# szy4017/DeepSense6G_TII

Hardware: NVIDIA B200
Metric: train samples/sec (fwd+bwd) (higher is better)
Workload: dtype bf16

## Files before the change

### deepsense6g_tii_b200/csrc/attn_api.cu

```cuda
#include <algorithm>
#include <atomic>

#include "tc_common.cuh"

namespace dsf {


__global__ void __launch_bounds__(256)
attn_delta_kernel(const __nv_bfloat16* __restrict__ y, const __nv_bfloat16* __restrict__ dy, float* __restrict__ delta, int B, int T,
                  int C, int nh) {
  pdl_trigger();
  pdl_wait();
  const int lane = threadIdx.x & 31;
  const int hs = C / nh, gl = hs / 8;
  const int nchunk = C / 8;
  for (int64_t row = (int64_t)blockIdx.x * 8 + (threadIdx.x >> 5); row < (int64_t)B * T; row += (int64_t)gridDim.x * 8) {
    const int b = (int)(row / T), t = (int)(row % T);
    for (int c0 = 0; c0 < nchunk; c0 += 32) {
      const int ch = c0 + lane;
      float acc = 0.f;
      if (ch < nchunk) {
        const uint4 a = __ldg(reinterpret_cast<const uint4*>(y + row * C + ch * 8));
        const uint4 d = __ldg(reinterpret_cast<const uint4*>(dy + row * C + ch * 8));
        const __nv_bfloat162* ap = reinterpret_cast<const __nv_bfloat162*>(&a);
        const __nv_bfloat162* dp = reinterpret_cast<const __nv_bfloat162*>(&d);
#pragma unroll
        for (int k = 0; k < 4; ++k) {
          const float2 af = __bfloat1622float2(ap[k]), df = __bfloat1622float2(dp[k]);
          acc += af.x * df.x + af.y * df.y;
        }
      }
      for (int o = gl >> 1; o > 0; o >>= 1) acc += __shfl_xor_sync(0xffffffffu, acc, o);
      if (ch < nchunk && (lane % gl) == 0) delta[((size_t)b * nh + (ch * 8) / hs) * T + t] = acc;
    }
  }
}

int attn_fwd_run(const void* qkv, void* y, float* lse, int B, int T, int C, int nh, const dsf_dropout* drop, uint32_t* bits, int force_nwg,
                 cudaStream_t st);
int attn_bwd_run(const void* qkv, const void* y, const void* dy, const float* lse, float* delta, void* dqkv, int B, int T, int C, int nh,
                 const dsf_dropout* drop, uint32_t* bits, int parts, cudaStream_t st);

int run_attn_delta(const void* y, const void* dy, float* delta, int B, int T, int C, int nh, cudaStream_t st) {
  launch_pdl(attn_delta_kernel, dim3(std::min(cdiv(B * T, 8), num_sms() * 8)), dim3(256), 0, st, (const __nv_bfloat16*)y, (const __nv_bfloat16*)dy,
             delta, B, T, C, nh);
  return check_launch("attn_bwd/delta");
}

static std::atomic<int> g_attn_impl{0};

}

using namespace dsf;

extern "C" int dsf_attn_set_impl(int32_t impl) {
  DSF_REQUIRE(impl >= 0 && impl <= 2, "attn_set_impl: impl must be 0 (default), 1 (128-row forward CTAs) or 2 (256-row forward CTAs)");
  g_attn_impl.store(impl, std::memory_order_relaxed);
  return DSF_OK;
}

static int check_attn_drop(const char* who, const dsf_dropout* drop, const uint32_t* bits, bool& on) {
  on = drop && drop->p > 0.f;
  if (!on) return DSF_OK;
  if (!(drop->p < 1.f)) { set_error("%s: dropout p must be in [0, 1)", who); return DSF_EINVAL; }
  if (!bits) { set_error("%s: attention dropout needs the drop_bits buffer", who); return DSF_EINVAL; }
  return DSF_OK;
}

static int check_head_size(const char* who, int hs) {
  if (hs == 16 || hs == 32 || hs == 64 || hs == 128) return DSF_OK;
  set_error("%s: head size %d not supported (16, 32, 64, 128)", who, hs);
  return DSF_EUNSUPPORTED;
}

extern "C" int64_t dsf_attn_drop_words(int32_t B, int32_t T, int32_t nh) {
  if (B <= 0 || T <= 0 || nh <= 0) return 0;
  return (int64_t)B * nh * T * (2 * cdiv(T, 64));
}

extern "C" int dsf_attn_fwd(const void* qkv, void* y, float* lse, int32_t B, int32_t T, int32_t C, int32_t nh, const dsf_dropout* drop,
                            uint32_t* drop_bits, void* stream) {
  DSF_REQUIRE(qkv && y && lse, "attn_fwd: NULL pointer");
  bool drop_on;
  if (int e = check_attn_drop("attn_fwd", drop, drop_bits, drop_on)) return e;
  DSF_REQUIRE(B > 0 && T > 0 && C > 0 && nh > 0 && C % nh == 0, "attn_fwd: bad shape B=%d T=%d C=%d nh=%d", B, T, C, nh);
  DSF_REQUIRE(aligned16(qkv) && aligned16(y), "attn_fwd: 16-byte alignment required");
  DSF_REQUIRE(B <= 65535 && nh <= 65535, "attn_fwd: grid too large");
  if (int e = check_head_size("attn_fwd", C / nh)) return e;
  return attn_fwd_run(qkv, y, lse, B, T, C, nh, drop_on ? drop : nullptr, drop_bits, g_attn_impl.load(std::memory_order_relaxed), (cudaStream_t)stream);
}

static int attn_bwd_impl(const void* qkv, const void* y, const void* dy, const float* lse, float* delta, void* dqkv, int32_t B, int32_t T,
                         int32_t C, int32_t nh, const dsf_dropout* drop, const uint32_t* drop_bits, int parts, void* stream) {
  DSF_REQUIRE(qkv && y && dy && lse && delta && dqkv, "attn_bwd: NULL pointer");
  bool drop_on;
  if (int e = check_attn_drop("attn_bwd", drop, drop_bits, drop_on)) return e;
  DSF_REQUIRE(B > 0 && T > 0 && C > 0 && nh > 0 && C % nh == 0, "attn_bwd: bad shape B=%d T=%d C=%d nh=%d", B, T, C, nh);
  DSF_REQUIRE(aligned16(qkv) && aligned16(y) && aligned16(dy) && aligned16(dqkv), "attn_bwd: 16-byte alignment required");
  DSF_REQUIRE(B <= 65535 && nh <= 65535, "attn_bwd: grid too large");
  if (int e = check_head_size("attn_bwd", C / nh)) return e;
  return attn_bwd_run(qkv, y, dy, lse, delta, dqkv, B, T, C, nh, drop_on ? drop : nullptr, const_cast<uint32_t*>(drop_bits), parts, (cudaStream_t)stream);
}

extern "C" int dsf_attn_bwd(const void* qkv, const void* y, const void* dy, const float* lse, float* delta, void* dqkv, int32_t B,
                            int32_t T, int32_t C, int32_t nh, const dsf_dropout* drop, const uint32_t* drop_bits, void* stream) {
  return attn_bwd_impl(qkv, y, dy, lse, delta, dqkv, B, T, C, nh, drop, drop_bits, 7, stream);
}

extern "C" int dsf_attn_bwd_parts(const void* qkv, const void* y, const void* dy, const float* lse, float* delta, void* dqkv, int32_t B,
                                  int32_t T, int32_t C, int32_t nh, const dsf_dropout* drop, const uint32_t* drop_bits, int32_t parts,
                                  void* stream) {
  DSF_REQUIRE(parts > 0 && parts <= 7, "attn_bwd_parts: parts must be a non-empty subset of {1 = delta, 2 = dK/dV, 4 = dQ}");
  return attn_bwd_impl(qkv, y, dy, lse, delta, dqkv, B, T, C, nh, drop, drop_bits, parts, stream);
}
```

### deepsense6g_tii_b200/csrc/attn_tc2.cu

```cuda
#include <algorithm>
#include <cstdlib>

#include "tc_common.cuh"

namespace dsf {

using namespace tc;

__device__ __forceinline__ void tma_load_3d(uint32_t dst, const CUtensorMap* m, uint32_t bar, int c0, int c1, int c2) {
  asm volatile(
      "cp.async.bulk.tensor.3d.shared::cluster.global.mbarrier::complete_tx::bytes [%0], [%1, {%3, %4, %5}], [%2];" ::"r"(dst),
      "l"(reinterpret_cast<uint64_t>(m)), "r"(bar), "r"(c0), "r"(c1), "r"(c2)
      : "memory");
}
#ifdef DSF_ATTN_TRACE
__device__ long long g_attn_trace[3][64][6];
#define TRACE(who, it, slot)                                                                               \
  do {                                                                                                     \
    if (blockIdx.x == 0 && blockIdx.y == 0 && blockIdx.z == 0 && (threadIdx.x & 31) == 0 && (it) < 64)     \
      g_attn_trace[who][it][slot] = clock64();                                                             \
  } while (0)
#else
#define TRACE(who, it, slot) do {} while (0)
#endif

__device__ __forceinline__ float ex2_approx(float x) {
  float y;
  asm("ex2.approx.ftz.f32 %0, %1;" : "=f"(y) : "f"(x));
  return y;
}
__device__ __forceinline__ uint64_t pack2(float lo, float hi) { uint64_t r; asm("mov.b64 %0, {%1, %2};" : "=l"(r) : "f"(lo), "f"(hi)); return r; }
__device__ __forceinline__ void unpack2(uint64_t v, float& lo, float& hi) { asm("mov.b64 {%0, %1}, %2;" : "=f"(lo), "=f"(hi) : "l"(v)); }
__device__ __forceinline__ uint64_t fma2(uint64_t a, uint64_t b, uint64_t c) { uint64_t d; asm("fma.rn.f32x2 %0, %1, %2, %3;" : "=l"(d) : "l"(a), "l"(b), "l"(c)); return d; }
__device__ __forceinline__ uint64_t add2(uint64_t a, uint64_t b) { uint64_t d; asm("add.rn.f32x2 %0, %1, %2;" : "=l"(d) : "l"(a), "l"(b)); return d; }
__device__ __forceinline__ uint64_t mul2(uint64_t a, uint64_t b) { uint64_t d; asm("mul.rn.f32x2 %0, %1, %2;" : "=l"(d) : "l"(a), "l"(b)); return d; }
__device__ __forceinline__ void ex2_poly2(uint64_t x, float& p0, float& p1) {
  float x0, x1;
  unpack2(x, x0, x1);
  const uint64_t xc = pack2(fmaxf(x0, -126.f), fmaxf(x1, -126.f));
  const uint64_t t = add2(xc, pack2(12582912.f, 12582912.f));
  const uint64_t r = add2(t, pack2(-12582912.f, -12582912.f));
  const uint64_t f = fma2(r, pack2(-1.f, -1.f), xc);
  uint64_t q = fma2(f, pack2(0.05517164617776871f, 0.05517164617776871f), pack2(0.2426111251115799f, 0.2426111251115799f));
  q = fma2(q, f, pack2(0.6932609677314758f, 0.6932609677314758f));
  q = fma2(q, f, pack2(0.9999280571937561f, 0.9999280571937561f));
  float q0, q1, t0, t1;
  unpack2(q, q0, q1);
  unpack2(t, t0, t1);
  p0 = __int_as_float(__float_as_int(q0) + (__float_as_int(t0) << 23));
  p1 = __int_as_float(__float_as_int(q1) + (__float_as_int(t1) << 23));
}

template <int POLY>
__device__ __forceinline__ uint64_t ex2_pair(uint64_t x, int j) {
  float p0, p1;
  if (POLY > 0 && (j % (POLY > 0 ? POLY : 1)) == POLY - 1) {
    ex2_poly2(x, p0, p1);
  } else {
    float x0, x1;
    unpack2(x, x0, x1);
    p0 = ex2_approx(x0);
    p1 = ex2_approx(x1);
  }
  return pack2(p0, p1);
}
__device__ __forceinline__ uint32_t pack_bf16x2_pair(uint64_t v) {
  float lo, hi;
  unpack2(v, lo, hi);
  return pack_bf16x2(lo, hi);
}

struct AttnDrop {
  uint32_t thresh8;
  float scale;
  uint32_t k0, k1, site;
  uint32_t* bits;
  int Tw;
  const unsigned long long* seed_dev;
};
__device__ __forceinline__ uint32_t attn_keep_word(const AttnDrop& a, uint64_t rowid, uint32_t word) {
  uint32_t out = 0;
  const uint32_t t4 = a.thresh8 * 0x01010101u;
#pragma unroll
  for (int c = 0; c < 2; ++c) {
    const uint4 r = philox4x32(a.k0, a.k1, (uint32_t)rowid, (uint32_t)(rowid >> 32), word * 2 + c, a.site);
    const uint32_t w[4] = {r.x, r.y, r.z, r.w};
#pragma unroll
    for (int k = 0; k < 4; ++k) {
      const uint32_t ge = __vcmpgeu4(w[k], t4) & 0x01010101u;
      out |= (((ge * 0x01020408u) >> 24) & 0xFu) << (c * 16 + k * 4);
    }
  }
  return out;
}
__device__ __forceinline__ void named_bar_sync(int id, int nthreads) {
  asm volatile("bar.sync %0, %1;" ::"r"(id), "r"(nthreads) : "memory");
}
__device__ __forceinline__ void named_bar_arrive(int id, int nthreads) {
  asm volatile("bar.arrive %0, %1;" ::"r"(id), "r"(nthreads) : "memory");
}

template <int HS>
struct HeadCfg {
  static constexpr int BOXC = HS < 64 ? HS : 64;
  static constexpr int ROWB = BOXC * 2;
  static constexpr int NHALF = HS / BOXC;
  static constexpr uint32_t SWZ = ROWB == 128 ? SWZ_128B : (ROWB == 64 ? SWZ_64B : SWZ_32B);
  static constexpr int KPH = ROWB / 32;
};

template <int HS>
__device__ __forceinline__ uint64_t kmaj_desc(uint32_t tile, int R, int kk) {
  using H = HeadCfg<HS>;
  const uint32_t off = (uint32_t)(kk / H::KPH) * R * H::ROWB + (uint32_t)(kk % H::KPH) * 32;
  return make_smem_desc(tile + off, 16, 8 * H::ROWB, H::SWZ);
}
template <int HS>
__device__ __forceinline__ uint64_t mnmaj_desc(uint32_t tile, int R, int kk) {
  using H = HeadCfg<HS>;
  return make_smem_desc(tile + (uint32_t)kk * 16 * H::ROWB, (uint32_t)R * H::ROWB, 8 * H::ROWB, H::SWZ);
}
template <int KC>
__device__ __forceinline__ uint64_t pdesc(uint32_t tile, int kk) {
  return make_smem_desc(tile + (uint32_t)kk * 256, 128, KC * 16, SWZ_NONE);
}

__device__ __forceinline__ void tc_commit_elect(uint32_t bar) {
  if (elect_one()) tc::tc_commit(bar);
  __syncwarp();
}
template <int HS>
__device__ __forceinline__ void mma_over_head(uint32_t tmem_d, uint32_t a_tile, int RA, uint32_t b_tile, int RB, uint32_t idesc) {
  using H = HeadCfg<HS>;
  const uint64_t da = make_smem_desc(a_tile, 16, 8 * H::ROWB, H::SWZ), db = make_smem_desc(b_tile, 16, 8 * H::ROWB, H::SWZ);
  if (elect_one()) {
#pragma unroll
    for (int kk = 0; kk < HS / 16; ++kk) {
      const uint32_t oa = (uint32_t)(kk / H::KPH) * RA * H::ROWB + (uint32_t)(kk % H::KPH) * 32;
      const uint32_t ob = (uint32_t)(kk / H::KPH) * RB * H::ROWB + (uint32_t)(kk % H::KPH) * 32;
      tc_mma_bf16(tmem_d, da + (oa >> 4), db + (ob >> 4), idesc, kk != 0);
    }
  }
  __syncwarp();
}
template <int HS, int KC>
__device__ __forceinline__ void mma_over_rows(uint32_t tmem_d, uint32_t p_tile, uint32_t b_tile, uint32_t idesc, bool accumulate) {
  using H = HeadCfg<HS>;
  const uint64_t dp = make_smem_desc(p_tile, 128, KC * 16, SWZ_NONE);
  const uint64_t db = make_smem_desc(b_tile, (uint32_t)KC * H::ROWB, 8 * H::ROWB, H::SWZ);
  const uint32_t acc = accumulate ? 1u : 0u;
  if (elect_one()) {
#pragma unroll
    for (int kk = 0; kk < KC / 16; ++kk)
      tc_mma_bf16(tmem_d, dp + (uint32_t)((kk * 256) >> 4), db + (uint32_t)((kk * 16 * H::ROWB) >> 4), idesc, kk == 0 ? acc : 1u);
  }
  __syncwarp();
}

template <int HS, int KC, int CW = 0>
__device__ __forceinline__ void mma_over_rows_ts(uint32_t tmem_d, uint32_t p_tmem, uint32_t b_tile, uint32_t idesc, bool accumulate) {
  using H = HeadCfg<HS>;
  const uint64_t db = make_smem_desc(b_tile, (uint32_t)KC * H::ROWB, 8 * H::ROWB, H::SWZ);
  const uint32_t acc = accumulate ? 1u : 0u;
  if (elect_one()) {
#pragma unroll
    for (int kk = 0; kk < KC / 16; ++kk) {
      const uint32_t col = CW > 0 ? (uint32_t)((kk * 16 / (CW > 0 ? CW : 1)) * CW + (kk * 16 % (CW > 0 ? CW : 1)) / 2) : (uint32_t)(kk * 8);
      tc_mma_bf16_ts(tmem_d, p_tmem + col, db + (uint32_t)((kk * 16 * H::ROWB) >> 4), idesc, kk == 0 ? acc : 1u);
    }
  }
  __syncwarp();
}

template <int HS>
__device__ __forceinline__ void mma_over_head_ts(uint32_t tmem_d, uint32_t a_tmem, uint32_t b_tile, int RB, uint32_t idesc) {
  using H = HeadCfg<HS>;
  const uint64_t db = make_smem_desc(b_tile, 16, 8 * H::ROWB, H::SWZ);
  if (elect_one()) {
#pragma unroll
    for (int kk = 0; kk < HS / 16; ++kk) {
      const uint32_t ob = (uint32_t)(kk / H::KPH) * RB * H::ROWB + (uint32_t)(kk % H::KPH) * 32;
      tc_mma_bf16_ts(tmem_d, a_tmem + (uint32_t)(kk * 8), db + (ob >> 4), idesc, kk != 0);
    }
  }
  __syncwarp();
}

template <int HS>
__device__ __forceinline__ void tma_tile(uint32_t dst, const CUtensorMap* m, uint32_t bar, int col0, int row0, int b, int R) {
  using H = HeadCfg<HS>;
#pragma unroll
  for (int hf = 0; hf < H::NHALF; ++hf) tma_load_3d(dst + hf * R * H::ROWB, m, bar, col0 + hf * H::BOXC, row0, b);
}

template <int KC>
__device__ __forceinline__ void store_p32(uint8_t* tile, int row, int c, const uint32_t (&pk)[16]) {
#pragma unroll
  for (int cc = 0; cc < 4; ++cc) {
    uint8_t* dst = tile + ((size_t)(row >> 3) * (KC / 8) + (c >> 3) + cc) * 128 + (row & 7) * 16;
    *reinterpret_cast<uint4*>(dst) = make_uint4(pk[4 * cc], pk[4 * cc + 1], pk[4 * cc + 2], pk[4 * cc + 3]);
  }
}

__device__ __forceinline__ void store_row16_bf16(__nv_bfloat16* dst, const uint32_t (&a)[16], float scale) {
#pragma unroll
  for (int e = 0; e < 16; e += 8)
    *reinterpret_cast<uint4*>(dst + e) =
        make_uint4(pack_bf16x2(__uint_as_float(a[e]) * scale, __uint_as_float(a[e + 1]) * scale),
                   pack_bf16x2(__uint_as_float(a[e + 2]) * scale, __uint_as_float(a[e + 3]) * scale),
                   pack_bf16x2(__uint_as_float(a[e + 4]) * scale, __uint_as_float(a[e + 5]) * scale),
                   pack_bf16x2(__uint_as_float(a[e + 6]) * scale, __uint_as_float(a[e + 7]) * scale));
}

template <int HS, int BQ, int ST, int NP>
struct BwdKV2 {
  static constexpr int KV_BYTES = 128 * HS * 2, Q_BYTES = BQ * HS * 2;
  static constexpr int K_OFF = 0, V_OFF = KV_BYTES, Q_OFF = 2 * KV_BYTES, DO_OFF = Q_OFF + ST * Q_BYTES;
  static constexpr int BAR_OFF = DO_OFF + ST * Q_BYTES;
  static constexpr int NBAR = 2 + 2 * ST + 4;
  static constexpr int STAT_OFF = BAR_OFF + NBAR * 8 + 16;
  static constexpr int THREADS = 256 * NP + 64;
  static_assert(4 * BQ + 2 * HS <= 512, "TMEM budget");
  static_assert(STAT_OFF % 16 == 0, "float4 reads of the statistics");
  static int dyn_bytes(int T) { return STAT_OFF + 2 * cdiv(T, BQ) * BQ * 4 + 1024; }
};

template <int HS, int BQ, int ST, int NP, bool DROP, int POLY>
__global__ void __launch_bounds__(256 * NP + 64, 1)
attn_bwd_kv2_kernel(const __grid_constant__ CUtensorMap tmKV, const __grid_constant__ CUtensorMap tmQ, const __grid_constant__ CUtensorMap tmDO,
                    const float* __restrict__ lse, const float* __restrict__ delta, __nv_bfloat16* __restrict__ dqkv, int T, int C, int nh,
                    float scale, AttnDrop ad) {
  using L = BwdKV2<HS, BQ, ST, NP>;
  constexpr int MMAW = 8 * NP, TMAW = 8 * NP + 1;
  extern __shared__ uint8_t smem_raw[];
  const uint32_t sbase = (smem_u32(smem_raw) + 1023u) & ~1023u;
  uint8_t* smem = smem_raw + (sbase - smem_u32(smem_raw));
  const uint32_t bar0 = sbase + L::BAR_OFF;
  const uint32_t kv_full = bar0, acc_done = bar0 + 8, q_full = bar0 + 16, q_empty = q_full + 8 * ST, s_full = q_empty + 8 * ST,
                 ds_full = s_full + 16, tmem_slot = ds_full + 16;
  const int warp = __shfl_sync(0xffffffffu, (int)(threadIdx.x >> 5), 0), lane = threadIdx.x & 31;
  const int kv0 = blockIdx.x * 128, h = blockIdx.y, b = blockIdx.z;
  const int n_q = (T + BQ - 1) / BQ;

  pdl_trigger();
  if (threadIdx.x == 0) {
    mbar_init(kv_full, 1);
    mbar_init(acc_done, 1);
    for (int s = 0; s < ST; ++s) { mbar_init(q_full + 8 * s, 1); mbar_init(q_empty + 8 * s, 1); }
    for (int w = 0; w < 2; ++w) { mbar_init(s_full + 8 * w, 1); mbar_init(ds_full + 8 * w, 256 * NP); }
    fence_barrier_init();
  }
  if (warp == MMAW) { tmem_alloc(tmem_slot, 512); tmem_relinquish(); }
  if (warp == TMAW && lane == 0) { tma_prefetch_desc(&tmKV); tma_prefetch_desc(&tmQ); tma_prefetch_desc(&tmDO); }
  tc_fence_before();
  __syncthreads();
  tc_fence_after();
  uint32_t tmem_base;
  asm volatile("ld.shared.b32 %0, [%1];" : "=r"(tmem_base) : "r"(tmem_slot));
  pdl_wait();
  const uint32_t tm_dv = tmem_base + 4 * BQ, tm_dk = tm_dv + HS;

  if (warp == TMAW) {
    if (lane == 0) {
      mbar_expect_tx(kv_full, 2 * L::KV_BYTES);
      tma_tile<HS>(sbase + L::K_OFF, &tmKV, kv_full, C + h * HS, kv0, b, 128);
      tma_tile<HS>(sbase + L::V_OFF, &tmKV, kv_full, 2 * C + h * HS, kv0, b, 128);
      for (int i = 0; i < n_q; ++i) {
        const int st = i % ST;
        if (i >= ST) mbar_wait(q_empty + 8 * st, ((i / ST) - 1) & 1);
        mbar_expect_tx(q_full + 8 * st, 2 * L::Q_BYTES);
        tma_tile<HS>(sbase + L::Q_OFF + st * L::Q_BYTES, &tmQ, q_full + 8 * st, h * HS, i * BQ, b, BQ);
        tma_tile<HS>(sbase + L::DO_OFF + st * L::Q_BYTES, &tmDO, q_full + 8 * st, h * HS, i * BQ, b, BQ);
      }
    }
  } else if (warp == MMAW) {
    {
      constexpr uint32_t idesc_s = make_idesc_bf16(128, BQ, 0, 0);
      constexpr uint32_t idesc_g = make_idesc_bf16(128, HS, 0, 1);
      mbar_wait(kv_full, 0);
      mbar_wait(q_full, 0);
      tc_fence_after();
      mma_over_head<HS>(tmem_base, sbase + L::K_OFF, 128, sbase + L::Q_OFF, BQ, idesc_s);
      mma_over_head<HS>(tmem_base + BQ, sbase + L::V_OFF, 128, sbase + L::DO_OFF, BQ, idesc_s);
      tc_commit_elect(s_full);
      for (int i = 0; i < n_q; ++i) {
        const int bf = i & 1, st = i % ST;
        TRACE(2, i, 0);
        if (i + 1 < n_q) {
          const int sn = (i + 1) % ST, bn = (i + 1) & 1;
          mbar_wait(q_full + 8 * sn, ((i + 1) / ST) & 1);
          TRACE(2, i, 1);
          tc_fence_after();
          mma_over_head<HS>(tmem_base + bn * 2 * BQ, sbase + L::K_OFF, 128, sbase + L::Q_OFF + sn * L::Q_BYTES, BQ, idesc_s);
          mma_over_head<HS>(tmem_base + bn * 2 * BQ + BQ, sbase + L::V_OFF, 128, sbase + L::DO_OFF + sn * L::Q_BYTES, BQ, idesc_s);
          tc_commit_elect(s_full + 8 * bn);
        }
        TRACE(2, i, 2);
        mbar_wait(ds_full + 8 * bf, (i >> 1) & 1);
        TRACE(2, i, 3);
        tc_fence_after();
        mma_over_rows_ts<HS, BQ, 32 / NP>(tm_dv, tmem_base + bf * 2 * BQ, sbase + L::DO_OFF + st * L::Q_BYTES, idesc_g, i > 0);
        mma_over_rows_ts<HS, BQ, 32 / NP>(tm_dk, tmem_base + bf * 2 * BQ + BQ, sbase + L::Q_OFF + st * L::Q_BYTES, idesc_g, i > 0);
        tc_commit_elect(q_empty + 8 * st);
        TRACE(2, i, 4);
      }
      tc_commit_elect(acc_done);
    }
  } else {
    constexpr int CW = BQ / (2 * NP);
    const int wgi = warp >> 2;
    const int row = (warp & 3) * 32 + lane;
    const uint32_t lane_off = (uint32_t)((warp & 3) * 32) << 16;
    const bool key_ok = (kv0 + row) < T;
    const float scale_log2 = scale * 1.4426950408889634f;
    const float* lse_g = lse + ((size_t)b * nh + h) * T;
    const float* delta_g = delta + ((size_t)b * nh + h) * T;
    static_assert(BQ == 64 && (CW == 32 || CW == 16), "a 64-query tile in 32- or 16-column shares");
    const size_t bh = (size_t)b * nh + h;
    const int kw = kv0 / 32 + (warp & 3);
    float* s_lse = reinterpret_cast<float*>(smem + L::STAT_OFF);
    float* s_delta = s_lse + n_q * BQ;
    for (int idx = threadIdx.x; idx < n_q * BQ; idx += 256 * NP) {
      s_lse[idx] = idx < T ? __ldg(lse_g + idx) * -1.4426950408889634f : -INFINITY;
      s_delta[idx] = idx < T ? -__ldg(delta_g + idx) : 0.f;
    }
    uint32_t wv = 0xFFFFFFFFu;
    auto fetch_w = [&](int it) {
      const int qq = it * BQ + wgi * CW + (lane % CW);
      wv = qq < T ? ad.bits[(bh * T + qq) * ad.Tw + kw] : 0u;
    };
    if (DROP) fetch_w(0);
    named_bar_sync(1, 256 * NP);
    for (int i = 0; i < n_q; ++i) {
      const int bf = i & 1;
      const float* wst = s_lse + i * BQ + wgi * CW;
      const float* wsd = s_delta + i * BQ + wgi * CW;
      const uint32_t myw = wv;
      if ((warp & 3) == 0 && wgi < 2) TRACE(wgi, i, 0);
      if (DROP && i + 1 < n_q) fetch_w(i + 1);
      if ((warp & 3) == 0 && wgi < 2) TRACE(wgi, i, 1);
      mbar_wait(s_full + 8 * bf, (i >> 1) & 1);
      if ((warp & 3) == 0 && wgi < 2) TRACE(wgi, i, 2);
      tc_fence_after();
      const uint32_t tm_s = tmem_base + bf * 2 * BQ + lane_off + wgi * CW, tm_dp = tm_s + BQ;
      uint32_t rs[CW], rp[CW];
      if constexpr (CW == 32) { tmem_ld32(tm_s, rs); tmem_ld32(tm_dp, rp); }
      else { tmem_ld16(tm_s, rs); tmem_ld16(tm_dp, rp); }
      tmem_wait_ld();
      if ((warp & 3) == 0 && wgi < 2) TRACE(wgi, i, 3);
      const uint64_t sc2 = pack2(scale_log2, scale_log2);
#pragma unroll
      for (int c = 0; c < CW; c += 16) {
        uint32_t pk[8], dk[8];
#pragma unroll
        for (int e = 0; e < 16; e += 4) {
          if (!DROP) {
            const ulonglong2 nl = *reinterpret_cast<const ulonglong2*>(wst + c + e);
            const ulonglong2 nd = *reinterpret_cast<const ulonglong2*>(wsd + c + e);
#pragma unroll
            for (int u = 0; u < 4; u += 2) {
              const uint64_t x = fma2(pack2(__uint_as_float(rs[c + e + u]), __uint_as_float(rs[c + e + u + 1])), sc2, u ? nl.y : nl.x);
              const uint64_t p2 = ex2_pair<POLY>(x, (c + e + u) / 2);
              const uint64_t t2 = add2(pack2(__uint_as_float(rp[c + e + u]), __uint_as_float(rp[c + e + u + 1])), u ? nd.y : nd.x);
              pk[(e + u) / 2] = pack_bf16x2_pair(p2);
              dk[(e + u) / 2] = pack_bf16x2_pair(mul2(p2, t2));
            }
            continue;
          }
          const float4 l4 = *reinterpret_cast<const float4*>(wst + c + e);
          const float4 d4 = *reinterpret_cast<const float4*>(wsd + c + e);
          const float ls[4] = {l4.x, l4.y, l4.z, l4.w}, dl[4] = {d4.x, d4.y, d4.z, d4.w};
          float p[4], d[4];
#pragma unroll
          for (int u = 0; u < 4; ++u) {
            p[u] = ex2_approx(fmaf(__uint_as_float(rs[c + e + u]), scale_log2, ls[u]));
            float dp = __uint_as_float(rp[c + e + u]);
            const float m = (__shfl_sync(0xffffffffu, myw, c + e + u) >> lane) & 1u ? ad.scale : 0.f;
            dp *= m;
            d[u] = p[u] * (dp + dl[u]);
            p[u] *= m;
          }
          pk[e / 2] = pack_bf16x2(p[0], p[1]);
          pk[e / 2 + 1] = pack_bf16x2(p[2], p[3]);
          dk[e / 2] = pack_bf16x2(d[0], d[1]);
          dk[e / 2 + 1] = pack_bf16x2(d[2], d[3]);
        }
        tmem_st8(tm_s + c / 2, pk);
        tmem_st8(tm_dp + c / 2, dk);
      }
      if ((warp & 3) == 0 && wgi < 2) TRACE(wgi, i, 4);
      tmem_wait_st();
      tc_fence_before();
      mbar_arrive(ds_full + 8 * bf);
      if ((warp & 3) == 0 && wgi < 2) TRACE(wgi, i, 5);
    }
    mbar_wait(acc_done, 0);
    tc_fence_after();
    const int ld = 3 * C;
    __nv_bfloat16* dk_row = dqkv + ((size_t)b * T + kv0 + row) * ld + C + h * HS;
    __nv_bfloat16* dv_row = dk_row + C;
    constexpr int NSPLIT = (NP == 2 && HS >= 32) ? 2 : 1;
    constexpr int CH = HS / NSPLIT;
    const int which = wgi & 1, part = wgi >> 1;
    if (part < NSPLIT) {
#pragma unroll 1
      for (int c = part * CH; c < (part + 1) * CH; c += 16) {
        uint32_t a[16];
        tmem_ld16((which == 0 ? tm_dk : tm_dv) + lane_off + c, a);
        tmem_wait_ld();
        if (key_ok) store_row16_bf16((which == 0 ? dk_row : dv_row) + c, a, which == 0 ? scale : 1.0f);
      }
    }
  }
  tc_fence_before();
  __syncthreads();
  if (warp == MMAW) tmem_dealloc(tmem_base, 512);
}

template <int HS, int ST>
struct BwdQ2 {
  static constexpr int BKV = 64;
  static constexpr int Q_BYTES = 128 * HS * 2, KV_BYTES = BKV * HS * 2;
  static constexpr int Q_OFF = 0, DO_OFF = Q_BYTES, K_OFF = 2 * Q_BYTES, V_OFF = K_OFF + ST * KV_BYTES;
  static constexpr int BAR_OFF = V_OFF + ST * KV_BYTES;
  static constexpr int NBAR = 2 + 2 * ST + 4;
  static constexpr int DYN = BAR_OFF + NBAR * 8 + 16 + 1024;
  static_assert(4 * BKV + HS <= 512, "TMEM budget");
};

template <int HS, int ST, bool AT, int NP, bool DROP, int POLY>
__global__ void __launch_bounds__(256 * NP + 64, 1)
attn_bwd_q2_kernel(const __grid_constant__ CUtensorMap tmQ, const __grid_constant__ CUtensorMap tmDO, const __grid_constant__ CUtensorMap tmKV,
                   const float* __restrict__ lse, const float* __restrict__ delta, __nv_bfloat16* __restrict__ dqkv, int T, int C, int nh,
                   float scale, AttnDrop ad, const __nv_bfloat16* __restrict__ qkv, const __nv_bfloat16* __restrict__ dy) {
  using L = BwdQ2<HS, ST>;
  constexpr int BKV = L::BKV;
  constexpr int MMAW = 8 * NP, TMAW = 8 * NP + 1;
  extern __shared__ uint8_t smem_raw[];
  const uint32_t sbase = (smem_u32(smem_raw) + 1023u) & ~1023u;
  const uint32_t bar0 = sbase + L::BAR_OFF;
  const uint32_t q_full = bar0, acc_done = bar0 + 8, kv_full = bar0 + 16, kv_empty = kv_full + 8 * ST, s_full = kv_empty + 8 * ST,
                 ds_full = s_full + 16, tmem_slot = ds_full + 16;
  const int warp = __shfl_sync(0xffffffffu, (int)(threadIdx.x >> 5), 0), lane = threadIdx.x & 31;
  const int q0 = blockIdx.x * 128, h = blockIdx.y, b = blockIdx.z;
  const int n_kv = (T + BKV - 1) / BKV;
  constexpr uint32_t TMEM_COLS = (4 * BKV + HS + (AT ? (HS >= 32 ? HS : 32) : 0)) <= 256 ? 256 : 512;
  static_assert(4 * BKV + 2 * HS <= 512, "TMEM budget (S/dP double-buffered, dQ, Q and dO rows)");

  pdl_trigger();
  if (threadIdx.x == 0) {
    mbar_init(q_full, AT ? 256 : 1);
    mbar_init(acc_done, 1);
    for (int s = 0; s < ST; ++s) { mbar_init(kv_full + 8 * s, 1); mbar_init(kv_empty + 8 * s, 1); }
    for (int w = 0; w < 2; ++w) { mbar_init(s_full + 8 * w, 1); mbar_init(ds_full + 8 * w, 256 * NP); }
    fence_barrier_init();
  }
  if (warp == MMAW) { tmem_alloc(tmem_slot, TMEM_COLS); tmem_relinquish(); }
  if (warp == TMAW && lane == 0) { tma_prefetch_desc(&tmKV); tma_prefetch_desc(&tmQ); tma_prefetch_desc(&tmDO); }
  tc_fence_before();
  __syncthreads();
  tc_fence_after();
  uint32_t tmem_base;
  asm volatile("ld.shared.b32 %0, [%1];" : "=r"(tmem_base) : "r"(tmem_slot));
  pdl_wait();
  const uint32_t tm_dq = tmem_base + 4 * BKV;
  const uint32_t tm_q = tm_dq + HS, tm_do = tm_q + (HS >= 32 ? HS / 2 : 16);

  if (warp == TMAW) {
    if (lane == 0) {
      if (!AT) {
        mbar_expect_tx(q_full, 2 * L::Q_BYTES);
        tma_tile<HS>(sbase + L::Q_OFF, &tmQ, q_full, h * HS, q0, b, 128);
        tma_tile<HS>(sbase + L::DO_OFF, &tmDO, q_full, h * HS, q0, b, 128);
      }
      for (int j = 0; j < n_kv; ++j) {
        const int st = j % ST;
        if (j >= ST) mbar_wait(kv_empty + 8 * st, ((j / ST) - 1) & 1);
        mbar_expect_tx(kv_full + 8 * st, 2 * L::KV_BYTES);
        tma_tile<HS>(sbase + L::K_OFF + st * L::KV_BYTES, &tmKV, kv_full + 8 * st, C + h * HS, j * BKV, b, BKV);
        tma_tile<HS>(sbase + L::V_OFF + st * L::KV_BYTES, &tmKV, kv_full + 8 * st, 2 * C + h * HS, j * BKV, b, BKV);
      }
    }
  } else if (warp == MMAW) {
    {
      constexpr uint32_t idesc_s = make_idesc_bf16(128, BKV, 0, 0);
      constexpr uint32_t idesc_q = make_idesc_bf16(128, HS, 0, 1);
      mbar_wait(q_full, 0);
      mbar_wait(kv_full, 0);
      tc_fence_after();
      if (AT) {
        mma_over_head_ts<HS>(tmem_base, tm_q, sbase + L::K_OFF, BKV, idesc_s);
        mma_over_head_ts<HS>(tmem_base + BKV, tm_do, sbase + L::V_OFF, BKV, idesc_s);
      } else {
        mma_over_head<HS>(tmem_base, sbase + L::Q_OFF, 128, sbase + L::K_OFF, BKV, idesc_s);
        mma_over_head<HS>(tmem_base + BKV, sbase + L::DO_OFF, 128, sbase + L::V_OFF, BKV, idesc_s);
      }
      tc_commit_elect(s_full);
      for (int j = 0; j < n_kv; ++j) {
        const int bf = j & 1, st = j % ST;
        if (j + 1 < n_kv) {
          const int sn = (j + 1) % ST, bn = (j + 1) & 1;
          mbar_wait(kv_full + 8 * sn, ((j + 1) / ST) & 1);
          tc_fence_after();
          if (AT) {
            mma_over_head_ts<HS>(tmem_base + bn * 2 * BKV, tm_q, sbase + L::K_OFF + sn * L::KV_BYTES, BKV, idesc_s);
            mma_over_head_ts<HS>(tmem_base + bn * 2 * BKV + BKV, tm_do, sbase + L::V_OFF + sn * L::KV_BYTES, BKV, idesc_s);
          } else {
            mma_over_head<HS>(tmem_base + bn * 2 * BKV, sbase + L::Q_OFF, 128, sbase + L::K_OFF + sn * L::KV_BYTES, BKV, idesc_s);
            mma_over_head<HS>(tmem_base + bn * 2 * BKV + BKV, sbase + L::DO_OFF, 128, sbase + L::V_OFF + sn * L::KV_BYTES, BKV, idesc_s);
          }
          tc_commit_elect(s_full + 8 * bn);
        }
        mbar_wait(ds_full + 8 * bf, (j >> 1) & 1);
        tc_fence_after();
        mma_over_rows_ts<HS, BKV, 32 / NP>(tm_dq, tmem_base + bf * 2 * BKV + BKV, sbase + L::K_OFF + st * L::KV_BYTES, idesc_q, j > 0);
        tc_commit_elect(kv_empty + 8 * st);
      }
      tc_commit_elect(acc_done);
    }
  } else {
    constexpr int CW = BKV / (2 * NP);
    static_assert(BKV == 64 && (CW == 32 || CW == 16), "a 64-key tile in 32- or 16-column shares");
    const int wgi = warp >> 2;
    const int row = (warp & 3) * 32 + lane;
    const uint32_t lane_off = (uint32_t)((warp & 3) * 32) << 16;
    const int q = q0 + row;
    const bool q_ok = q < T;
    const float scale_log2 = scale * 1.4426950408889634f;
    const float my_lse = q_ok ? lse[((size_t)b * nh + h) * T + q] * 1.4426950408889634f : INFINITY;
    const float my_delta = q_ok ? delta[((size_t)b * nh + h) * T + q] : 0.f;
    if (AT && wgi < 2) {
      const __nv_bfloat16* src = wgi == 0 ? qkv + ((size_t)b * T + q) * (3 * C) + h * HS : dy + ((size_t)b * T + q) * C + h * HS;
      const uint32_t dst = (wgi == 0 ? tm_q : tm_do) + lane_off;
#pragma unroll 1
      for (int c = 0; c < HS; c += 32) {
        uint32_t wds[16];
#pragma unroll
        for (int k = 0; k < 4; ++k) {
          const bool real = q_ok && (HS >= 32 || k < 2);
          const uint4 v = real ? __ldg(reinterpret_cast<const uint4*>(src + c) + k) : make_uint4(0u, 0u, 0u, 0u);
          wds[4 * k] = v.x; wds[4 * k + 1] = v.y; wds[4 * k + 2] = v.z; wds[4 * k + 3] = v.w;
        }
        tmem_st16(dst + c / 2, wds);
      }
      tmem_wait_st();
      tc_fence_before();
      mbar_arrive(q_full);
    }
    const uint32_t* my_bits = (DROP && q_ok) ? ad.bits + (((size_t)b * nh + h) * T + q) * ad.Tw + (wgi * CW) / 32 : nullptr;
    uint32_t wnext = my_bits ? my_bits[0] : 0xFFFFFFFFu;
    for (int j = 0; j < n_kv; ++j) {
      const int bf = j & 1, kv0 = j * BKV;
      const uint32_t keepw = wnext >> ((wgi * CW) % 32);
      if (my_bits && j + 1 < n_kv) wnext = my_bits[2 * (j + 1)];
      mbar_wait(s_full + 8 * bf, (j >> 1) & 1);
      tc_fence_after();
      const uint32_t tm_s = tmem_base + bf * 2 * BKV + lane_off + wgi * CW, tm_dp = tm_s + BKV;
      const bool full = kv0 + BKV <= T;
      uint32_t rs[CW], rp[CW];
      if constexpr (CW == 32) { tmem_ld32(tm_s, rs); tmem_ld32(tm_dp, rp); }
      else { tmem_ld16(tm_s, rs); tmem_ld16(tm_dp, rp); }
      tmem_wait_ld();
#pragma unroll
      for (int c = 0; c < CW; c += 16) {
        uint32_t dk[8];
        if (full && !DROP) {
          const uint64_t sc2 = pack2(scale_log2, scale_log2), nl2 = pack2(-my_lse, -my_lse), nd2 = pack2(-my_delta, -my_delta);
#pragma unroll
          for (int e = 0; e < 16; e += 2) {
            const uint64_t x = fma2(pack2(__uint_as_float(rs[c + e]), __uint_as_float(rs[c + e + 1])), sc2, nl2);
            const uint64_t p2 = ex2_pair<POLY>(x, (c + e) / 2);
            const uint64_t t2 = add2(pack2(__uint_as_float(rp[c + e]), __uint_as_float(rp[c + e + 1])), nd2);
            dk[e / 2] = pack_bf16x2_pair(mul2(p2, t2));
          }
        } else {
          const int k0 = kv0 + wgi * CW + c;
#pragma unroll
          for (int e = 0; e < 16; e += 2) {
            float p0 = (k0 + e < T) ? ex2_approx(fmaf(__uint_as_float(rs[c + e]), scale_log2, -my_lse)) : 0.f;
            float p1 = (k0 + e + 1 < T) ? ex2_approx(fmaf(__uint_as_float(rs[c + e + 1]), scale_log2, -my_lse)) : 0.f;
            float dp0 = __uint_as_float(rp[c + e]), dp1 = __uint_as_float(rp[c + e + 1]);
            if (DROP) {
              dp0 *= (keepw >> (c + e)) & 1u ? ad.scale : 0.f;
              dp1 *= (keepw >> (c + e + 1)) & 1u ? ad.scale : 0.f;
            }
            dk[e / 2] = pack_bf16x2(p0 * (dp0 - my_delta), p1 * (dp1 - my_delta));
          }
        }
        tmem_st8(tm_dp + c / 2, dk);
      }
      tmem_wait_st();
      tc_fence_before();
      mbar_arrive(ds_full + 8 * bf);
    }
    mbar_wait(acc_done, 0);
    tc_fence_after();
    __nv_bfloat16* dq_row = dqkv + ((size_t)b * T + q) * (3 * C) + h * HS;
    constexpr int NG = (HS / 16) < 2 * NP ? (HS / 16) : 2 * NP;
    constexpr int CH = HS / NG;
    const int g = wgi;
    if (g < NG) {
#pragma unroll 1
      for (int c = g * CH; c < (g + 1) * CH; c += 16) {
        uint32_t a[16];
        tmem_ld16(tm_dq + lane_off + c, a);
        tmem_wait_ld();
        if (q_ok) store_row16_bf16(dq_row + c, a, scale);
      }
    }
  }
  tc_fence_before();
  __syncthreads();
  if (warp == MMAW) tmem_dealloc(tmem_base, TMEM_COLS);
}

template <int HS, int KST, int VST, int NWG = 2, bool PT = false>
struct Fwd3 {
  static constexpr int BKV = 64;
  static constexpr int Q_BYTES = 128 * HS * 2, KV_BYTES = BKV * HS * 2, P_BYTES = 128 * BKV * 2;
  static constexpr int Q_OFF = 0, K_OFF = NWG * Q_BYTES, V_OFF = K_OFF + KST * KV_BYTES, P_OFF = V_OFF + VST * KV_BYTES;
  static constexpr int BAR_OFF = P_OFF + (PT ? 0 : 2 * NWG * P_BYTES);
  static constexpr int NBAR = 1 + 2 * KST + 2 * VST + 12;
  static constexpr int DYN = BAR_OFF + NBAR * 8 + 16 + 1024;
  static constexpr int THREADS = 128 * NWG + 64;
  static constexpr int MIN_CTAS = NWG == 1 ? 2 : 1;
  static constexpr uint32_t TMEM_COLS = NWG == 1 ? 256 : 512;
  static_assert(2 * NWG * BKV + NWG * HS <= (int)TMEM_COLS, "TMEM budget");
  static_assert(DYN <= 232448 / MIN_CTAS - 1024 * (MIN_CTAS - 1), "shared memory budget");
};

template <int HS, int KST, int VST, bool PT, bool PP, int NWG = 2, int POLY = 0>
__global__ void __launch_bounds__(128 * NWG + 64, NWG == 1 ? 2 : 1)
attn_fwd3_kernel(const __grid_constant__ CUtensorMap tmQ, const __grid_constant__ CUtensorMap tmKV, __nv_bfloat16* __restrict__ y,
                 float* __restrict__ lse, int T, int C, int nh, float scale_log2, AttnDrop ad) {
  using L = Fwd3<HS, KST, VST, NWG, PT>;
  constexpr int BKV = L::BKV;
  constexpr int MMAW = 4 * NWG, TMAW = 4 * NWG + 1;
  static_assert(!PP || NWG == 2, "ping-pong needs two warpgroups");
  extern __shared__ uint8_t smem_raw[];
  const uint32_t sbase = (smem_u32(smem_raw) + 1023u) & ~1023u;
  uint8_t* smem = smem_raw + (sbase - smem_u32(smem_raw));
  const uint32_t bar0 = sbase + L::BAR_OFF;
  const uint32_t q_full = bar0, k_full = bar0 + 8, k_empty = k_full + 8 * KST, v_full = k_empty + 8 * KST, v_empty = v_full + 8 * VST,
                 s_full = v_empty + 8 * VST, p_full = s_full + 32, p_empty = p_full + 32, tmem_slot = p_empty + 32;
  const int warp = __shfl_sync(0xffffffffu, (int)(threadIdx.x >> 5), 0), lane = threadIdx.x & 31;
  const int q0 = blockIdx.x * (128 * NWG), h = blockIdx.y, b = blockIdx.z;
  const int n_kv = (T + BKV - 1) / BKV;

  pdl_trigger();
  if (threadIdx.x == 0) {
    mbar_init(q_full, 1);
    for (int s = 0; s < KST; ++s) { mbar_init(k_full + 8 * s, 1); mbar_init(k_empty + 8 * s, 1); }
    for (int s = 0; s < VST; ++s) { mbar_init(v_full + 8 * s, 1); mbar_init(v_empty + 8 * s, 1); }
    for (int i = 0; i < 2 * NWG; ++i) { mbar_init(s_full + 8 * i, 1); mbar_init(p_full + 8 * i, 128); mbar_init(p_empty + 8 * i, 1); }
    fence_barrier_init();
  }
  if (warp == MMAW) { tmem_alloc(tmem_slot, L::TMEM_COLS); tmem_relinquish(); }
  if (warp == TMAW && lane == 0) { tma_prefetch_desc(&tmQ); tma_prefetch_desc(&tmKV); }
  tc_fence_before();
  __syncthreads();
  tc_fence_after();
  uint32_t tmem_base;
  asm volatile("ld.shared.b32 %0, [%1];" : "=r"(tmem_base) : "r"(tmem_slot));
  pdl_wait();
  if (ad.thresh8 && ad.seed_dev != nullptr) {
    const unsigned long long sd = __ldg(ad.seed_dev);
    ad.k0 ^= (uint32_t)(sd & 0xFFFFFFFFull);
    ad.k1 ^= (uint32_t)(sd >> 32);
  }

  if (warp == TMAW) {
    if (lane == 0) {
      mbar_expect_tx(q_full, NWG * L::Q_BYTES);
      for (int w = 0; w < NWG; ++w) tma_tile<HS>(sbase + L::Q_OFF + w * L::Q_BYTES, &tmQ, q_full, h * HS, q0 + 128 * w, b, 128);
      for (int j = 0; j < n_kv; ++j) {
        const int ks = j % KST, vs = j % VST;
        if (j >= KST) mbar_wait(k_empty + 8 * ks, ((j / KST) - 1) & 1);
        mbar_expect_tx(k_full + 8 * ks, L::KV_BYTES);
        tma_tile<HS>(sbase + L::K_OFF + ks * L::KV_BYTES, &tmKV, k_full + 8 * ks, C + h * HS, j * BKV, b, BKV);
        if (j >= VST) mbar_wait(v_empty + 8 * vs, ((j / VST) - 1) & 1);
        mbar_expect_tx(v_full + 8 * vs, L::KV_BYTES);
        tma_tile<HS>(sbase + L::V_OFF + vs * L::KV_BYTES, &tmKV, v_full + 8 * vs, 2 * C + h * HS, j * BKV, b, BKV);
      }
    }
  } else if (warp == MMAW) {
    {
      constexpr uint32_t idesc_s = make_idesc_bf16(128, BKV, 0, 0);
      constexpr uint32_t idesc_o = make_idesc_bf16(128, HS, 0, 1);
      mbar_wait(q_full, 0);
      for (int jj = 0; jj < 2 && jj < n_kv; ++jj) {
        mbar_wait(k_full + 8 * (jj % KST), (jj / KST) & 1);
        tc_fence_after();
        for (int w = 0; w < NWG; ++w) {
          mma_over_head<HS>(tmem_base + (w * 2 + jj) * BKV, sbase + L::Q_OFF + w * L::Q_BYTES, 128, sbase + L::K_OFF + (jj % KST) * L::KV_BYTES,
                            BKV, idesc_s);
          tc_commit_elect(s_full + 8 * (w * 2 + jj));
        }
        tc_commit_elect(k_empty + 8 * (jj % KST));
      }
      for (int j = 0; j < n_kv; ++j) {
        const int buf = j & 1, vs = j % VST;
        TRACE(2, j, 0);
        mbar_wait(v_full + 8 * vs, (j / VST) & 1);
        for (int w = 0; w < NWG; ++w) {
          const int sb = w * 2 + buf;
          TRACE(2, j, 1 + 2 * w);
          mbar_wait(p_full + 8 * sb, (j >> 1) & 1);
          TRACE(2, j, 2 + 2 * w);
          tc_fence_after();
          if (PT)
            mma_over_rows_ts<HS, BKV>(tmem_base + 2 * NWG * BKV + w * HS, tmem_base + sb * BKV, sbase + L::V_OFF + vs * L::KV_BYTES, idesc_o, j > 0);
          else
            mma_over_rows<HS, BKV>(tmem_base + 2 * NWG * BKV + w * HS, sbase + L::P_OFF + sb * L::P_BYTES, sbase + L::V_OFF + vs * L::KV_BYTES, idesc_o,
                                   j > 0);
          tc_commit_elect(p_empty + 8 * sb);
          if (w == NWG - 1) tc_commit_elect(v_empty + 8 * vs);
          if (j + 2 < n_kv) {
            const int ks = (j + 2) % KST;
            if (w == 0) { mbar_wait(k_full + 8 * ks, ((j + 2) / KST) & 1); tc_fence_after(); }
            mma_over_head<HS>(tmem_base + sb * BKV, sbase + L::Q_OFF + w * L::Q_BYTES, 128, sbase + L::K_OFF + ks * L::KV_BYTES, BKV, idesc_s);
            tc_commit_elect(s_full + 8 * sb);
            if (w == NWG - 1) tc_commit_elect(k_empty + 8 * ks);
          }
        }
      }
    }
  } else {
    const int w = warp >> 2;
    const int row = (warp & 3) * 32 + lane;
    const uint32_t lane_off = (uint32_t)((warp & 3) * 32) << 16;
    const uint32_t tm_o = tmem_base + 2 * NWG * BKV + w * HS + lane_off;
    float m_run = -INFINITY, l_run = 0.f;
    if (PP && w == 1) named_bar_arrive(3, 256);
    for (int j = 0; j < n_kv; ++j) {
      const int kv0 = j * BKV, buf = j & 1, sb = w * 2 + buf;
      const uint32_t tm_s = tmem_base + sb * BKV + lane_off;
      uint8_t* p_tile = smem + L::P_OFF + sb * L::P_BYTES;
      if ((warp & 3) == 0) TRACE(w, j, 0);
      mbar_wait(s_full + 8 * sb, (j >> 1) & 1);
      if ((warp & 3) == 0) TRACE(w, j, 1);
      tc_fence_after();
      uint32_t r0[32], r1[32];
      tmem_ld32(tm_s, r0);
      tmem_ld32(tm_s + 32, r1);
      tmem_wait_ld();
      if ((warp & 3) == 0) TRACE(w, j, 2);
      float p_max = -INFINITY;
      if (kv0 + BKV <= T) {
        float m4[4] = {-INFINITY, -INFINITY, -INFINITY, -INFINITY};
#pragma unroll
        for (int i = 0; i < 32; ++i) m4[i & 3] = fmaxf(m4[i & 3], fmaxf(__uint_as_float(r0[i]), __uint_as_float(r1[i])));
        p_max = fmaxf(fmaxf(m4[0], m4[1]), fmaxf(m4[2], m4[3]));
      } else {
#pragma unroll
        for (int i = 0; i < 32; ++i) {
          if (kv0 + i < T) p_max = fmaxf(p_max, __uint_as_float(r0[i]));
          if (kv0 + 32 + i < T) p_max = fmaxf(p_max, __uint_as_float(r1[i]));
        }
      }
      p_max *= scale_log2;
      const bool need = p_max > m_run + 8.f;
      if (__any_sync(0xffffffffu, need)) {
        const float m_new = need ? p_max : m_run;
        const float alpha = ex2_approx(m_run - m_new);
        if (j > 0) {
          mbar_wait(p_empty + 8 * (w * 2 + ((j - 1) & 1)), ((j - 1) >> 1) & 1);
          tc_fence_after();
#pragma unroll 1
          for (int c = 0; c < HS; c += 16) {
            uint32_t o[16];
            tmem_ld16(tm_o + c, o);
            tmem_wait_ld();
#pragma unroll
            for (int i = 0; i < 16; ++i) o[i] = __float_as_uint(__uint_as_float(o[i]) * alpha);
            tmem_st16(tm_o + c, o);
          }
          tmem_wait_st();
        }
        l_run *= alpha;
        m_run = m_new;
      }
      if ((warp & 3) == 0) TRACE(w, j, 3);
      if (!PT && j >= 2) mbar_wait(p_empty + 8 * sb, ((j >> 1) - 1) & 1);
      if (PP) named_bar_sync(3 + w, 256);
      if ((warp & 3) == 0) TRACE(w, j, 4);
      float l_add = 0.f;
      const bool full = kv0 + BKV <= T;
      const int qrow = q0 + 128 * w + row;
      const uint64_t rowid = ((uint64_t)b * nh + h) * T + qrow;
      if (POLY > 0 && PT && full && !ad.thresh8) {
        const uint64_t sc2 = pack2(scale_log2, scale_log2), nm2 = pack2(-m_run, -m_run);
        uint64_t lsum = pack2(0.f, 0.f);
#pragma unroll
        for (int half = 0; half < 2; ++half) {
          uint32_t pk[16];
#pragma unroll
          for (int i = 0; i < 32; i += 2) {
            const uint32_t a0 = half ? r1[i] : r0[i], a1 = half ? r1[i + 1] : r0[i + 1];
            const uint64_t x = fma2(pack2(__uint_as_float(a0), __uint_as_float(a1)), sc2, nm2);
            float p0, p1;
            if (((i / 2) % (POLY > 0 ? POLY : 1)) == POLY - 1) {
              ex2_poly2(x, p0, p1);
            } else {
              float x0, x1;
              unpack2(x, x0, x1);
              p0 = ex2_approx(x0);
              p1 = ex2_approx(x1);
            }
            lsum = add2(lsum, pack2(p0, p1));
            pk[i / 2] = pack_bf16x2(p0, p1);
          }
          tmem_st16(tm_s + half * 16, pk);
        }
        float l0, l1;
        unpack2(lsum, l0, l1);
        l_add = l0 + l1;
      } else
#pragma unroll
      for (int half = 0; half < 2; ++half) {
        uint32_t keepw = 0xFFFFFFFFu;
        if (ad.thresh8) {
          keepw = attn_keep_word(ad, rowid, (uint32_t)(kv0 / 32 + half));
          if (qrow < T) ad.bits[rowid * ad.Tw + kv0 / 32 + half] = keepw;
        }
        uint32_t pk[16];
#pragma unroll
        for (int i = 0; i < 32; i += 2) {
          const uint32_t a0 = half ? r1[i] : r0[i], a1 = half ? r1[i + 1] : r0[i + 1];
          float p0 = ex2_approx(fmaf(__uint_as_float(a0), scale_log2, -m_run));
          float p1 = ex2_approx(fmaf(__uint_as_float(a1), scale_log2, -m_run));
          if (!full) {
            if (kv0 + half * 32 + i >= T) p0 = 0.f;
            if (kv0 + half * 32 + i + 1 >= T) p1 = 0.f;
          }
          l_add += p0 + p1;
          if (ad.thresh8) {
            p0 *= (keepw >> i) & 1u ? ad.scale : 0.f;
            p1 *= (keepw >> (i + 1)) & 1u ? ad.scale : 0.f;
          }
          pk[i / 2] = pack_bf16x2(p0, p1);
        }
        if (PT) tmem_st16(tm_s + half * 16, pk);
        else store_p32<BKV>(p_tile, row, half * 32, pk);
      }
      if (PP) named_bar_arrive(4 - w, 256);
      l_run += l_add;
      if (PT) tmem_wait_st();
      else fence_proxy_async();
      tc_fence_before();
      mbar_arrive(p_full + 8 * sb);
      if ((warp & 3) == 0) TRACE(w, j, 5);
    }
    mbar_wait(p_empty + 8 * (w * 2 + ((n_kv - 1) & 1)), ((n_kv - 1) >> 1) & 1);
    tc_fence_after();
    const int q = q0 + 128 * w + row;
    const float inv_l = 1.0f / l_run;
    __nv_bfloat16* yrow = y + ((size_t)b * T + q) * C + h * HS;
#pragma unroll 1
    for (int c = 0; c < HS; c += 16) {
      uint32_t o[16];
      tmem_ld16(tm_o + c, o);
      tmem_wait_ld();
      if (q < T) store_row16_bf16(yrow + c, o, inv_l);
    }
    if (q < T) lse[((size_t)b * nh + h) * T + q] = (m_run + log2f(l_run)) * 0.6931471805599453f;
  }
  tc_fence_before();
  __syncthreads();
  if (warp == MMAW) tmem_dealloc(tmem_base, L::TMEM_COLS);
}

typedef CUresult (*PFN_encodeTiled)(CUtensorMap*, CUtensorMapDataType, cuuint32_t, void*, const cuuint64_t*, const cuuint64_t*,
                                    const cuuint32_t*, const cuuint32_t*, CUtensorMapInterleave, CUtensorMapSwizzle,
                                    CUtensorMapL2promotion, CUtensorMapFloatOOBfill);
static PFN_encodeTiled get_encode3() {
  static PFN_encodeTiled fn = nullptr;
  if (!fn) {
    void* p = nullptr;
    cudaDriverEntryPointQueryResult q;
    if (cudaGetDriverEntryPoint("cuTensorMapEncodeTiled", &p, cudaEnableDefault, &q) == cudaSuccess && q == cudaDriverEntryPointSuccess)
      fn = (PFN_encodeTiled)p;
  }
  return fn;
}

static int make_tmap3(CUtensorMap* m, const void* base, int ncols, int T, int B, int box_cols, int box_rows) {
  PFN_encodeTiled enc = get_encode3();
  if (!enc) { set_error("cuTensorMapEncodeTiled entry point not available"); return DSF_ELAUNCH; }
  cuuint64_t gdim[3] = {(cuuint64_t)ncols, (cuuint64_t)T, (cuuint64_t)B};
  cuuint64_t gstr[2] = {(cuuint64_t)ncols * 2, (cuuint64_t)ncols * 2 * (cuuint64_t)T};
  cuuint32_t box[3] = {(cuuint32_t)box_cols, (cuuint32_t)box_rows, 1u};
  cuuint32_t estr[3] = {1u, 1u, 1u};
  CUtensorMapSwizzle sw = box_cols * 2 == 128 ? CU_TENSOR_MAP_SWIZZLE_128B : (box_cols * 2 == 64 ? CU_TENSOR_MAP_SWIZZLE_64B : CU_TENSOR_MAP_SWIZZLE_32B);
  CUresult r = enc(m, CU_TENSOR_MAP_DATA_TYPE_BFLOAT16, 3, const_cast<void*>(base), gdim, gstr, box, estr, CU_TENSOR_MAP_INTERLEAVE_NONE, sw,
                   CU_TENSOR_MAP_L2_PROMOTION_L2_256B, CU_TENSOR_MAP_FLOAT_OOB_FILL_NONE);
  if (r != CUDA_SUCCESS) { set_error("cuTensorMapEncodeTiled(3d) failed (%d) ncols=%d T=%d B=%d box=%dx%d", (int)r, ncols, T, B, box_cols, box_rows); return DSF_ELAUNCH; }
  return DSF_OK;
}

static const bool g_attn_exp_poly = getenv("DSF_ATTN_EXP_POLY") ? atoi(getenv("DSF_ATTN_EXP_POLY")) != 0 : true;

template <int HS, int KST, int VST, int NWG, int POLY>
static int launch_fwd3p(const void* qkv, void* y, float* lse, int B, int T, int C, int nh, const AttnDrop& ad, cudaStream_t st) {
  using L = Fwd3<HS, KST, VST, NWG, true>;
  using H = HeadCfg<HS>;
  static bool configured_on[64] = {};
  bool& configured = per_device_flag(configured_on);
  if (!configured) {
    if (cudaFuncSetAttribute(attn_fwd3_kernel<HS, KST, VST, true, false, NWG, POLY>, cudaFuncAttributeMaxDynamicSharedMemorySize, L::DYN) != cudaSuccess)
      return check_launch("attn_fwd3/attr");
    configured = true;
  }
  CUtensorMap tmQ, tmKV;
  if (int e = make_tmap3(&tmQ, qkv, 3 * C, T, B, H::BOXC, 128)) return e;
  if (int e = make_tmap3(&tmKV, qkv, 3 * C, T, B, H::BOXC, L::BKV)) return e;
  const float scale_log2 = (1.0f / sqrtf((float)HS)) * 1.4426950408889634f;
  dim3 grid(cdiv(T, 128 * NWG), nh, B);
  launch_pdl(attn_fwd3_kernel<HS, KST, VST, true, false, NWG, POLY>, grid, dim3(L::THREADS), L::DYN, st, tmQ, tmKV, (__nv_bfloat16*)y, lse, T, C, nh,
             scale_log2, ad);
  return check_launch("attn_fwd3");
}

template <int HS, int KST, int VST, int NWG>
static int launch_fwd3(const void* qkv, void* y, float* lse, int B, int T, int C, int nh, const AttnDrop& ad, cudaStream_t st) {
  if constexpr (NWG == 1) {
    if (g_attn_exp_poly) return launch_fwd3p<HS, KST, VST, NWG, (HS >= 128 ? 4 : 3)>(qkv, y, lse, B, T, C, nh, ad, st);
  }
  return launch_fwd3p<HS, KST, VST, NWG, 0>(qkv, y, lse, B, T, C, nh, ad, st);
}

int run_attn_delta(const void* y, const void* dy, float* delta, int B, int T, int C, int nh, cudaStream_t st);

static const bool g_attn_a_in_tmem = getenv("DSF_ATTN_A_TMEM") ? atoi(getenv("DSF_ATTN_A_TMEM")) != 0 : true;
constexpr int kBwdPairs = 1;

template <int HS, int BQ, int STA, int NP, bool DROP, int POLY>
static int launch_bwd_kv(const CUtensorMap& tmKV128, const CUtensorMap& tmQs, const CUtensorMap& tmDOs, const float* lse, const float* delta, void* dqkv,
                         dim3 grid, int T, int C, int nh, float scale, const AttnDrop& ad, cudaStream_t st) {
  using LA = BwdKV2<HS, BQ, STA, NP>;
  const int dyn = LA::dyn_bytes(T);
  if (dyn > 232448) { set_error("attn_bwd: T = %d needs %d bytes of shared memory for the per-query statistics (limit 232448)", T, dyn); return DSF_EUNSUPPORTED; }
  static bool configured_on[64] = {};
  bool& configured = per_device_flag(configured_on);
  if (!configured) {
    if (cudaFuncSetAttribute(attn_bwd_kv2_kernel<HS, BQ, STA, NP, DROP, POLY>, cudaFuncAttributeMaxDynamicSharedMemorySize, 232448) != cudaSuccess)
      return check_launch("attn_bwd2/kv/attr");
    configured = true;
  }
  launch_pdl(attn_bwd_kv2_kernel<HS, BQ, STA, NP, DROP, POLY>, grid, dim3(LA::THREADS), dyn, st, tmKV128, tmQs, tmDOs, lse, delta, (__nv_bfloat16*)dqkv, T, C,
             nh, scale, ad);
  return check_launch("attn_bwd2/kv");
}

template <int HS, int STB, bool AT, int NP, bool DROP, int POLY>
static int launch_bwd_q(const CUtensorMap& tmQ128, const CUtensorMap& tmDO128, const CUtensorMap& tmKV64, const float* lse, const float* delta, void* dqkv,
                        dim3 grid, int T, int C, int nh, float scale, const AttnDrop& ad, const void* qkv, const void* dy, cudaStream_t st) {
  using LB = BwdQ2<HS, STB>;
  static bool configured_on[64] = {};
  bool& configured = per_device_flag(configured_on);
  if (!configured) {
    if (cudaFuncSetAttribute(attn_bwd_q2_kernel<HS, STB, AT, NP, DROP, POLY>, cudaFuncAttributeMaxDynamicSharedMemorySize, LB::DYN) != cudaSuccess)
      return check_launch("attn_bwd2/q/attr");
    configured = true;
  }
  launch_pdl(attn_bwd_q2_kernel<HS, STB, AT, NP, DROP, POLY>, grid, dim3(256 * NP + 64), LB::DYN, st, tmQ128, tmDO128, tmKV64, lse, delta, (__nv_bfloat16*)dqkv, T,
             C, nh, scale, ad, (const __nv_bfloat16*)qkv, (const __nv_bfloat16*)dy);
  return check_launch("attn_bwd2/q");
}

template <int HS, int BQ, int STA, int STB>
static int launch_bwd2(const void* qkv, const void* y, const void* dy, const float* lse, float* delta, void* dqkv, int B, int T, int C, int nh,
                       const AttnDrop& ad, int parts, cudaStream_t st) {
  using H = HeadCfg<HS>;
  const float scale = 1.0f / sqrtf((float)HS);
  if (parts & 1) {
    if (int e = run_attn_delta(y, dy, delta, B, T, C, nh, st)) return e;
  }
  const dim3 grid(cdiv(T, 128), nh, B);
  const bool drop = ad.thresh8 != 0;
  if (parts & 2) {
    CUtensorMap tmKV128, tmQs, tmDOs;
    if (int e = make_tmap3(&tmKV128, qkv, 3 * C, T, B, H::BOXC, 128)) return e;
    if (int e = make_tmap3(&tmQs, qkv, 3 * C, T, B, H::BOXC, BQ)) return e;
    if (int e = make_tmap3(&tmDOs, dy, C, T, B, H::BOXC, BQ)) return e;
#define DSF_KV(DROP) launch_bwd_kv<HS, BQ, STA, kBwdPairs, DROP, 0>(tmKV128, tmQs, tmDOs, lse, (const float*)delta, dqkv, grid, T, C, nh, scale, ad, st)
    if (int e = drop ? DSF_KV(true) : DSF_KV(false)) return e;
#undef DSF_KV
  }
  if (parts & 4) {
    CUtensorMap tmQ128, tmDO128, tmKV64;
    if (int e = make_tmap3(&tmQ128, qkv, 3 * C, T, B, H::BOXC, 128)) return e;
    if (int e = make_tmap3(&tmDO128, dy, C, T, B, H::BOXC, 128)) return e;
    if (int e = make_tmap3(&tmKV64, qkv, 3 * C, T, B, H::BOXC, 64)) return e;
#define DSF_Q(AT, DROP) launch_bwd_q<HS, STB, AT, kBwdPairs, DROP, 0>(tmQ128, tmDO128, tmKV64, lse, (const float*)delta, dqkv, grid, T, C, nh, scale, ad, qkv, dy, st)
    int e;
    if (g_attn_a_in_tmem) e = drop ? DSF_Q(true, true) : DSF_Q(true, false);
    else e = drop ? DSF_Q(false, true) : DSF_Q(false, false);
#undef DSF_Q
    if (e) return e;
  }
  return DSF_OK;
}

#ifdef DSF_ATTN_TRACE
}
extern "C" int dsf_debug_attn_trace(long long* host_out) {
  return cudaMemcpyFromSymbol(host_out, dsf::g_attn_trace, sizeof(dsf::g_attn_trace)) == cudaSuccess ? 0 : 2;
}
namespace dsf {
#endif

static AttnDrop make_attn_drop(const dsf_dropout* d, uint32_t* bits, int T) {
  AttnDrop a{0u, 1.0f, 0u, 0u, 0u, bits, 2 * cdiv(T, 64), nullptr};
  if (d && d->p > 0.f && bits) {
    int k = (int)lrintf(d->p * 256.0f);
    k = std::max(1, std::min(255, k));
    a.thresh8 = (uint32_t)k;
    a.scale = 256.0f / (256.0f - (float)k);
    a.k0 = (uint32_t)(d->seed & 0xFFFFFFFFull) ^ d->step;
    a.k1 = (uint32_t)(d->seed >> 32);
    a.site = d->site;
    a.seed_dev = reinterpret_cast<const unsigned long long*>(d->seed_dev);
  }
  return a;
}

int attn_fwd_run(const void* qkv, void* y, float* lse, int B, int T, int C, int nh, const dsf_dropout* drop, uint32_t* bits, int force_nwg,
                 cudaStream_t st) {
  const AttnDrop ad = make_attn_drop(drop, bits, T);
  if (force_nwg != 2) {
    switch (C / nh) {
      case 16: return launch_fwd3<16, 3, 2, 1>(qkv, y, lse, B, T, C, nh, ad, st);
      case 32: return launch_fwd3<32, 3, 2, 1>(qkv, y, lse, B, T, C, nh, ad, st);
      case 64: return launch_fwd3<64, 3, 2, 1>(qkv, y, lse, B, T, C, nh, ad, st);
      case 128: return launch_fwd3<128, 2, 2, 1>(qkv, y, lse, B, T, C, nh, ad, st);
    }
  }
  switch (C / nh) {
    case 16: return launch_fwd3<16, 3, 2, 2>(qkv, y, lse, B, T, C, nh, ad, st);
    case 32: return launch_fwd3<32, 3, 2, 2>(qkv, y, lse, B, T, C, nh, ad, st);
    case 64: return launch_fwd3<64, 3, 2, 2>(qkv, y, lse, B, T, C, nh, ad, st);
    case 128: return launch_fwd3<128, 3, 2, 2>(qkv, y, lse, B, T, C, nh, ad, st);
  }
  set_error("attn_fwd: head size %d not supported (16, 32, 64, 128)", C / nh);
  return DSF_EUNSUPPORTED;
}

int attn_bwd_run(const void* qkv, const void* y, const void* dy, const float* lse, float* delta, void* dqkv, int B, int T, int C, int nh,
                 const dsf_dropout* drop, uint32_t* bits, int parts, cudaStream_t st) {
  const AttnDrop ad = make_attn_drop(drop, bits, T);
  switch (C / nh) {
    case 16: return launch_bwd2<16, 64, 3, 3>(qkv, y, dy, lse, delta, dqkv, B, T, C, nh, ad, parts, st);
    case 32: return launch_bwd2<32, 64, 3, 3>(qkv, y, dy, lse, delta, dqkv, B, T, C, nh, ad, parts, st);
    case 64: return launch_bwd2<64, 64, 3, 3>(qkv, y, dy, lse, delta, dqkv, B, T, C, nh, ad, parts, st);
    case 128: return launch_bwd2<128, 64, 3, 3>(qkv, y, dy, lse, delta, dqkv, B, T, C, nh, ad, parts, st);
  }
  set_error("attn_bwd: head size %d not supported (16, 32, 64, 128)", C / nh);
  return DSF_EUNSUPPORTED;
}

}
```

### deepsense6g_tii_b200/functional.py

```python
import math
import os

import torch
from torch.autograd.function import once_differentiable

from . import _capi as K
from ._capi import EPI_ACCUM, EPI_BIAS, EPI_RELU, EPI_RESIDUAL, GemmF32Desc

PER_BLOCK = ("ln1.weight", "ln1.bias", "ln2.weight", "ln2.bias",
             "attn.key.weight", "attn.key.bias", "attn.query.weight", "attn.query.bias",
             "attn.value.weight", "attn.value.bias", "attn.proj.weight", "attn.proj.bias",
             "mlp.0.weight", "mlp.0.bias", "mlp.2.weight", "mlp.2.bias")


def param_names(n_layer):
    names = ["pos_emb"]
    for i in range(n_layer):
        names += ["blocks.%d.%s" % (i, n) for n in PER_BLOCK]
    return names + ["ln_f.weight", "ln_f.bias"]


def _f32_linear_desc(M, N, Kd, flags, trans=None):
    return GemmF32Desc(M, N, Kd, 1, 1, 0, 0, Kd, 1, 0, 0, Kd, 1, 0, 0, N, 1, 1.0, flags)


class _Ctx:
    pass


_SIDE_STREAMS = {}


def _side_stream(device, which=0):
    key = (device.type, device.index, which)
    if key not in _SIDE_STREAMS:
        _SIDE_STREAMS[key] = torch.cuda.Stream(device=device)
    return _SIDE_STREAMS[key]


def _chain_mode(C, env, default):
    try:
        m = int(os.environ.get(env, default))
    except ValueError:
        m = default
    return (m >= 1 and C == 64) or (m >= 2 and C == 128)


def drop_site(kind, block=0):
    return 0 if kind == "embd" else 1 + 3 * block + ("attn", "proj", "mlp").index(kind)


class _Runner:

    def __init__(self, B, S, V, A_h, A_w, C, H, W, n_head, n_layer, feat_dtype, compute_dtype, layout):
        self.B, self.S, self.V, self.A_h, self.A_w, self.C, self.H, self.W = B, S, V, A_h, A_w, C, H, W
        self.nh, self.L = n_head, n_layer
        self.hs = C // n_head
        self.Tm = (V + 2) * S * A_h * A_w
        self.T = self.Tm + 2
        self.M = B * self.T
        self.bf16 = compute_dtype == torch.bfloat16
        self.act = torch.bfloat16 if self.bf16 else torch.float32
        self.grad_hook = None
        self.dropout = None
        self.shadows = None
        self.capture = None
        if self.bf16:
            if C % 64 != 0 or self.hs not in (16, 32, 64, 128):
                raise RuntimeError("bf16 tensor-core mode needs n_embd %% 64 == 0 and head size in {16,32,64,128}; "
                                   "got n_embd=%d n_head=%d" % (C, n_head))
        self.geom = K.make_geom(B, S, V, A_h, A_w, C, H, W, K.DSF_BF16 if feat_dtype == torch.bfloat16 else K.DSF_F32, layout)

    def _linear_fwd(self, x, w, b, out_dtype, relu=False, residual=None):
        M, Kd = x.shape
        N = w.shape[0]
        out = torch.empty(M, N, device=x.device, dtype=out_dtype)
        flags = EPI_BIAS | (EPI_RELU if relu else 0) | (EPI_RESIDUAL if residual is not None else 0)
        K.gemm_f32(_f32_linear_desc(M, N, Kd, flags), x, w, out, bias=b, residual=residual)
        return out

    def _linear_bwd(self, dy, x, w):
        M, N = dy.shape
        Kd = x.shape[1]
        dev = dy.device
        dw = torch.zeros(N, Kd, device=dev, dtype=torch.float32)
        db = torch.zeros(N, device=dev, dtype=torch.float32)
        K.colsum(dy, db)
        K.gemm_f32(GemmF32Desc(N, Kd, M, 1, 1, 0, 0, 1, N, 0, 0, 1, Kd, 0, 0, Kd, 1, 1.0, 0), dy, x, dw)
        dx = torch.empty(M, Kd, device=dev, dtype=torch.float32)
        K.gemm_f32(GemmF32Desc(M, Kd, N, 1, 1, 0, 0, N, 1, 0, 0, 1, Kd, 0, 0, Kd, 1, 1.0, 0), dy, w, dx)
        return dx, dw, db

    def _attn_fwd(self, qkv, st):
        B, T, C, nh, hs = self.B, self.T, self.C, self.nh, self.hs
        dev = qkv.device
        y = torch.empty(self.M, C, device=dev, dtype=self.act)
        if self.bf16:
            st.lse = torch.empty(B, nh, T, device=dev, dtype=torch.float32)
            K.attn_fwd(qkv, y, st.lse, B, T, C, nh)
            return y
        P = torch.empty(B, nh, T, T, device=dev, dtype=torch.float32)
        q, k, v = qkv, qkv[:, C:], qkv[:, 2 * C:]
        ld = 3 * C
        K.gemm_f32(GemmF32Desc(T, T, hs, B, nh, T * ld, hs, ld, 1, T * ld, hs, ld, 1, nh * T * T, T * T, T, 1,
                               1.0 / math.sqrt(hs), 0), q, k, P)
        K.softmax_fwd(P, B * nh * T, T)
        K.gemm_f32(GemmF32Desc(T, hs, T, B, nh, nh * T * T, T * T, T, 1, T * ld, hs, 1, ld, T * C, hs, C, 1, 1.0, 0), P, v, y)
        st.P = P
        return y

    def _attn_bwd(self, dy, qkv, y, st):
        B, T, C, nh, hs = self.B, self.T, self.C, self.nh, self.hs
        dev = dy.device
        dqkv = torch.empty(self.M, 3 * C, device=dev, dtype=self.act)
        if self.bf16:
            delta = torch.empty(B, nh, T, device=dev, dtype=torch.float32)
            K.attn_bwd(qkv, y, dy, st.lse, delta, dqkv, B, T, C, nh)
            return dqkv
        P = st.P
        q, k, v = qkv, qkv[:, C:], qkv[:, 2 * C:]
        dq, dk, dv = dqkv, dqkv[:, C:], dqkv[:, 2 * C:]
        ld = 3 * C
        sc = 1.0 / math.sqrt(hs)
        dP = torch.empty_like(P)
        K.gemm_f32(GemmF32Desc(T, T, hs, B, nh, T * C, hs, C, 1, T * ld, hs, ld, 1, nh * T * T, T * T, T, 1, 1.0, 0), dy, v, dP)
        K.gemm_f32(GemmF32Desc(T, hs, T, B, nh, nh * T * T, T * T, 1, T, T * C, hs, 1, C, T * ld, hs, ld, 1, 1.0, 0), P, dy, dv)
        K.softmax_bwd(dP, P, B * nh * T, T)
        K.gemm_f32(GemmF32Desc(T, hs, T, B, nh, nh * T * T, T * T, T, 1, T * ld, hs, 1, ld, T * ld, hs, ld, 1, sc, 0), dP, k, dq)
        K.gemm_f32(GemmF32Desc(T, hs, T, B, nh, nh * T * T, T * T, 1, T, T * ld, hs, 1, ld, T * ld, hs, ld, 1, sc, 0), dP, q, dk)
        return dqkv

    def forward(self, feats, gps_emb, params, residual=True):
        if self.bf16:
            return self._forward_bf16(feats, gps_emb, params, residual)
        dev = gps_emb.device
        M, C, L = self.M, self.C, self.L
        f32 = torch.float32
        saved = _Ctx()
        saved.layers = []
        x = torch.empty(M, C, device=dev, dtype=f32)
        K.tokens_fwd(self.geom, feats[0], feats[1], feats[2], gps_emb, params[0], x)
        saved.shadows = []
        for i in range(L):
            (ln1w, ln1b, ln2w, ln2b, kw, kb, qw, qb, vw, vb, pw, pb, w1, b1, w2, b2) = params[1 + 16 * i: 17 + 16 * i]
            st = _Ctx()
            wqkv = torch.cat([qw, kw, vw], dim=0)
            bqkv = torch.cat([qb, kb, vb], dim=0)
            st.wqkv = wqkv
            st.x_in = x
            st.mean1 = torch.empty(M, device=dev, dtype=f32)
            st.rstd1 = torch.empty(M, device=dev, dtype=f32)
            st.h1 = torch.empty(M, C, device=dev, dtype=f32)
            K.layernorm_fwd(x, ln1w, ln1b, st.h1, st.mean1, st.rstd1)
            st.qkv = self._linear_fwd(st.h1, wqkv, bqkv, f32)
            st.y = self._attn_fwd(st.qkv, st)
            x_mid = self._linear_fwd(st.y, pw, pb, f32, residual=x)
            st.x_mid = x_mid
            st.mean2 = torch.empty(M, device=dev, dtype=f32)
            st.rstd2 = torch.empty(M, device=dev, dtype=f32)
            st.h2 = torch.empty(M, C, device=dev, dtype=f32)
            K.layernorm_fwd(x_mid, ln2w, ln2b, st.h2, st.mean2, st.rstd2)
            st.a = self._linear_fwd(st.h2, w1, b1, f32, relu=True)
            if self.capture is not None:
                self.capture["relu.%d" % i] = st.a
            x = self._linear_fwd(st.a, w2, b2, f32, residual=x_mid)
            saved.layers.append(st)
        saved.x_last = x
        saved.mean_f = torch.empty(M, device=dev, dtype=f32)
        saved.rstd_f = torch.empty(M, device=dev, dtype=f32)
        yf = torch.empty(M, C, device=dev, dtype=f32)
        K.layernorm_fwd(x, params[-2], params[-1], yf, saved.mean_f, saved.rstd_f)
        outs = [torch.empty_like(f) for f in feats]
        K.upsample_add_fwd(self.geom, yf, feats if residual else [torch.zeros_like(f) for f in feats], outs)
        gps_out = yf.view(self.B, self.T, C)[:, self.Tm:, :].contiguous()
        return outs, gps_out, saved

    def _forward_bf16(self, feats, gps_emb, params, residual):
        dev = gps_emb.device
        M, C, L = self.M, self.C, self.L
        f32, bf = torch.float32, torch.bfloat16
        F = params[13].shape[0] if L > 0 else 4 * C
        saved = _Ctx()
        saved.layers = []
        env = os.environ.get("DSF_WGRAD_STREAM")
        use_side = (env == "1") if env in ("0", "1") else torch.cuda.is_current_stream_capturing()
        main = torch.cuda.current_stream()
        side = _side_stream(dev) if use_side else None
        sizes = [3 * C * C, 3 * C * C, C * C, C * C, F * C, F * C, C * F, C * F]
        packed = []

        def pack(i):
            (ln1w, ln1b, ln2w, ln2b, kw, kb, qw, qb, vw, vb, pw, pb, w1, b1, w2, b2) = params[1 + 16 * i: 17 + 16 * i]
            st = _Ctx()
            if self.shadows is not None:
                v = self.shadows["views"][i]
                st.wqkv, st.wqkv_t, st.wp, st.wp_t, st.w1, st.w1_t, st.w2, st.w2_t, st.bqkv = (
                    v["wqkv"], v["wqkv_t"], v["wp"], v["wp_t"], v["w1"], v["w1_t"], v["w2"], v["w2_t"], v["bqkv"])
                if not self.shadows["fresh"]:
                    K.pack_block_weights(qw, kw, vw, pw, w1, w2, qb, kb, vb,
                                         (st.wqkv, st.wqkv_t, st.wp, st.wp_t, st.w1, st.w1_t, st.w2, st.w2_t, st.bqkv))
                return st
            flat = torch.empty(sum(sizes), device=dev, dtype=bf)
            views, off = [], 0
            for n in sizes:
                views.append(flat[off:off + n])
                off += n
            st.wqkv, st.wqkv_t = views[0].view(3 * C, C), views[1].view(C, 3 * C)
            st.wp, st.wp_t = views[2].view(C, C), views[3].view(C, C)
            st.w1, st.w1_t = views[4].view(F, C), views[5].view(C, F)
            st.w2, st.w2_t = views[6].view(C, F), views[7].view(F, C)
            st.bqkv = torch.empty(3 * C, device=dev, dtype=f32)
            K.pack_block_weights(qw, kw, vw, pw, w1, w2, qb, kb, vb,
                                 (st.wqkv, st.wqkv_t, st.wp, st.wp_t, st.w1, st.w1_t, st.w2, st.w2_t, st.bqkv))
            return st

        if side is not None:
            ev = torch.cuda.Event()
            ev.record(main)
            side.wait_event(ev)
            with torch.cuda.stream(side):
                for i in range(L):
                    st = pack(i)
                    st.packed_ev = torch.cuda.Event()
                    st.packed_ev.record(side)
                    packed.append(st)
        x = torch.empty(M, C, device=dev, dtype=f32)
        K.tokens_fwd(self.geom, feats[0], feats[1], feats[2], gps_emb, params[0], x)
        if self._drop("embd") is not None:
            K.dropout_inplace(x, self._drop("embd"))
        def take(i):
            if side is not None:
                st = packed[i]
                main.wait_event(st.packed_ev)
                st.packed_ev = None
                return st
            return pack(i)

        chain = _chain_mode(C, "DSF_CHAIN", 2) and F == 4 * C and L > 0 and self.dropout is None
        yf = torch.empty(M, C, device=dev, dtype=f32)
        saved.mean_f = torch.empty(M, device=dev, dtype=f32)
        saved.rstd_f = torch.empty(M, device=dev, dtype=f32)
        nxt = None
        for i in range(L):
            (ln1w, ln1b, ln2w, ln2b, kw, kb, qw, qb, vw, vb, pw, pb, w1, b1, w2, b2) = params[1 + 16 * i: 17 + 16 * i]
            st = take(i) if nxt is None else nxt
            nxt = None
            bqkv = st.bqkv
            st.x_in = x
            if not hasattr(st, "h1"):
                stats = torch.empty(2, M, device=dev, dtype=f32)
                st.mean1, st.rstd1 = stats[0], stats[1]
                st.h1 = torch.empty(M, C, device=dev, dtype=bf)
                K.layernorm_fwd(x, ln1w, ln1b, st.h1, st.mean1, st.rstd1)
                st.qkv = torch.empty(M, 3 * C, device=dev, dtype=bf)
                K.gemm_bf16_nt(st.h1, st.wqkv, st.qkv, bias=bqkv)
            stats2 = torch.empty(2, M, device=dev, dtype=f32)
            st.mean2, st.rstd2 = stats2[0], stats2[1]
            st.y = torch.empty(M, C, device=dev, dtype=bf)
            st.lse = torch.empty(self.B, self.nh, self.T, device=dev, dtype=f32)
            st.drop_bits = None
            if self._drop("attn", i) is not None:
                st.drop_bits = torch.empty(K.attn_drop_words(self.B, self.T, self.nh), device=dev, dtype=torch.int32)
                if "capture" in self.dropout:
                    self.dropout["capture"]["attn_bits.%d" % i] = st.drop_bits
            K.attn_fwd(st.qkv, st.y, st.lse, self.B, self.T, C, self.nh, self._drop("attn", i), st.drop_bits)
            st.x_mid = torch.empty(M, C, device=dev, dtype=f32)
            st.h2 = torch.empty(M, C, device=dev, dtype=bf)
            st.a = torch.empty(M, F, device=dev, dtype=bf)
            x_new = torch.empty(M, C, device=dev, dtype=f32)
            if chain:
                if i + 1 < L:
                    sn = take(i + 1)
                    statn = torch.empty(2, M, device=dev, dtype=f32)
                    sn.mean1, sn.rstd1 = statn[0], statn[1]
                    sn.h1 = torch.empty(M, C, device=dev, dtype=bf)
                    sn.qkv = torch.empty(M, 3 * C, device=dev, dtype=bf)
                    K.chain_fwd(st.y, x, st.wp, st.w1, st.w2, sn.wqkv, pb, b1, b2, sn.bqkv, ln2w, ln2b, params[1 + 16 * (i + 1)],
                                params[2 + 16 * (i + 1)], st.x_mid, x_new, st.h2, st.a, sn.h1, sn.qkv, None, st.mean2, st.rstd2, sn.mean1, sn.rstd1)
                    nxt = sn
                else:
                    K.chain_fwd(st.y, x, st.wp, st.w1, st.w2, None, pb, b1, b2, None, ln2w, ln2b, params[-2], params[-1], st.x_mid, x_new,
                                st.h2, st.a, None, None, yf, st.mean2, st.rstd2, saved.mean_f, saved.rstd_f)
            else:
                K.gemm_bf16_nt(st.y, st.wp, st.x_mid, bias=pb, residual=x, drop=self._drop("proj", i))
                K.layernorm_fwd(st.x_mid, ln2w, ln2b, st.h2, st.mean2, st.rstd2)
                K.gemm_bf16_nt(st.h2, st.w1, st.a, bias=b1, relu=True)
                K.gemm_bf16_nt(st.a, st.w2, x_new, bias=b2, residual=st.x_mid, drop=self._drop("mlp", i))
            if self.capture is not None:
                self.capture["relu.%d" % i] = st.a
            x = x_new
            saved.layers.append(st)
        saved.x_last = x
        if not chain:
            K.layernorm_fwd(x, params[-2], params[-1], yf, saved.mean_f, saved.rstd_f)
        outs = [torch.empty_like(f) for f in feats]
        K.upsample_add_fwd(self.geom, yf, feats if residual else [torch.zeros_like(f) for f in feats], outs)
        gps_out = yf.view(self.B, self.T, C)[:, self.Tm:, :].contiguous()
        if self.shadows is not None and not self.shadows["fresh"]:
            self.shadows["owner"].mark_shadows_fresh()
        return outs, gps_out, saved

    def _drop(self, kind, block=0):
        d = self.dropout
        if d is None:
            return None
        p = float(d.get("resid" if kind in ("proj", "mlp") else kind, 0.0))
        if p <= 0.0:
            return None
        sd = d.get("seed_dev")
        return K.Dropout(p, int(d["seed"]), drop_site(kind, block), int(d.get("step", 0)), None if sd is None else sd.data_ptr())

    def _backward_bf16(self, saved, params, douts, dgps_out, residual):
        dev = douts[0].device
        M, C, L = self.M, self.C, self.L
        f32, bf = torch.float32, torch.bfloat16
        grads = [None] * len(params)
        dyf = torch.empty(M, C, device=dev, dtype=f32)
        K.upsample_add_bwd(self.geom, douts, dgps_out, dyf)
        F = params[13].shape[0] if L > 0 else 4 * C
        sizes = [3 * C * C, C * C, F * C, C * F, 3 * C, C, F, C, C, C, C, C]
        per_block = sum(sizes)
        gbuf = torch.zeros(L * per_block + 2 * C + self.T * C, device=dev, dtype=f32)

        def block_views(i):
            out, off = [], i * per_block
            for n in sizes:
                out.append(gbuf[off:off + n])
                off += n
            return out

        def bucket(i):
            return gbuf[i * per_block:(i + 1) * per_block + (2 * C if i == L - 1 else 0)]

        env = os.environ.get("DSF_WGRAD_STREAM")
        use_side = (env == "1") if env in ("0", "1") else torch.cuda.is_current_stream_capturing()
        main = torch.cuda.current_stream()
        side = _side_stream(dev) if use_side else None
        side_q = _side_stream(dev, 1) if use_side else None

        def fork(fn, stream=None):
            stream = stream or side
            if stream is None:
                fn()
                return
            ev = torch.cuda.Event()
            ev.record(main)
            stream.wait_event(ev)
            with torch.cuda.stream(stream):
                fn()

        def join(stream=None):
            stream = stream or side
            if stream is not None:
                ev = torch.cuda.Event()
                ev.record(stream)
                main.wait_event(ev)

        pending = None

        def join_pending():
            nonlocal pending
            if pending is not None:
                ev, blk, _keep = pending
                main.wait_event(ev)
                pending = None
                if self.grad_hook is not None:
                    self.grad_hook.block_ready(blk, bucket(blk))

        dgf, dbf = gbuf[L * per_block:L * per_block + C], gbuf[L * per_block + C:L * per_block + 2 * C]
        dh_dt = bf if os.environ.get("DSF_LN_DY_BF16", "1") == "1" else f32
        dx = torch.empty(M, C, device=dev, dtype=f32)
        dxa_bufs = [torch.empty(M, C, device=dev, dtype=bf), torch.empty(M, C, device=dev, dtype=bf)]
        last = block_views(L - 1) if L > 0 else None
        K.layernorm_bwd(dyf, saved.x_last, params[-2], saved.mean_f, saved.rstd_f, None, dx, dgf, dbf,
                        dx_bf16=dxa_bufs[(L - 1) & 1] if L > 0 else None, dx_colsum=last[7] if L > 0 else None,
                        byprod_drop=self._drop("mlp", L - 1) if L > 0 else None)
        grads[-2], grads[-1] = dgf, dbf
        for i in reversed(range(L)):
            base = 1 + 16 * i
            (ln1w, ln1b, ln2w, ln2b, kw, kb, qw, qb, vw, vb, pw, pb, w1, b1, w2, b2) = params[base: base + 16]
            st = saved.layers[i]
            dxa = dxa_bufs[i & 1]
            dwqkv, dwp, dw1, dw2, dbqkv, dbp, db1, db2, dg1, dbt1, dg2, dbt2 = block_views(i)
            dwqkv, dwp, dw1, dw2 = dwqkv.view(3 * C, C), dwp.view(C, C), dw1.view(F, C), dw2.view(C, F)
            fork(lambda: K.gemm_bf16_tn(dxa, st.a, dw2))
            da = torch.empty(M, F, device=dev, dtype=bf)
            K.gemm_bf16_nt(dxa, st.w2_t, da, relu_src=st.a)

            fork(lambda: K.gemm_bf16_tn(da, st.h2, dw1, colsum=db1))
            dh2 = torch.empty(M, C, device=dev, dtype=dh_dt)
            K.gemm_bf16_nt(da, st.w1_t, dh2)
            dx_mid = torch.empty(M, C, device=dev, dtype=f32)
            dxm = torch.empty(M, C, device=dev, dtype=bf)
            K.layernorm_bwd(dh2, st.x_mid, ln2w, st.mean2, st.rstd2, dx, dx_mid, dg2, dbt2, dx_bf16=dxm, dx_colsum=dbp,
                            byprod_drop=self._drop("proj", i))
            fork(lambda: K.gemm_bf16_tn(dxm, st.y, dwp))
            dy = torch.empty(M, C, device=dev, dtype=bf)
            K.gemm_bf16_nt(dxm, st.wp_t, dy)
            dqkv = torch.empty(M, 3 * C, device=dev, dtype=bf)
            delta = torch.empty(self.B, self.nh, self.T, device=dev, dtype=f32)
            if side is None:
                K.attn_bwd(st.qkv, st.y, dy, st.lse, delta, dqkv, self.B, self.T, C, self.nh, self._drop("attn", i), st.drop_bits)
            else:
                adrop = self._drop("attn", i)
                K.attn_bwd(st.qkv, st.y, dy, st.lse, delta, dqkv, self.B, self.T, C, self.nh, adrop, st.drop_bits, parts=1)
                fork(lambda: K.attn_bwd(st.qkv, st.y, dy, st.lse, delta, dqkv, self.B, self.T, C, self.nh, adrop, st.drop_bits, parts=4), side_q)
                K.attn_bwd(st.qkv, st.y, dy, st.lse, delta, dqkv, self.B, self.T, C, self.nh, adrop, st.drop_bits, parts=2)
                join(side_q)

            fork(lambda: K.gemm_bf16_tn(dqkv, st.h1, dwqkv, colsum=dbqkv))
            dh1 = torch.empty(M, C, device=dev, dtype=dh_dt)
            K.gemm_bf16_nt(dqkv, st.wqkv_t, dh1)
            join_pending()
            if side is not None:
                ev_blk = torch.cuda.Event()
                ev_blk.record(side)
                pending = (ev_blk, i, (st, da, dxm, dqkv))
            dx = torch.empty(M, C, device=dev, dtype=f32)
            prev = block_views(i - 1) if i > 0 else None
            K.layernorm_bwd(dh1, st.x_in, ln1w, st.mean1, st.rstd1, dx_mid, dx, dg1, dbt1,
                            dx_bf16=dxa_bufs[(i - 1) & 1] if i > 0 else None, dx_colsum=prev[7] if i > 0 else None,
                            byprod_drop=self._drop("mlp", i - 1) if i > 0 else None)
            grads[base: base + 16] = [dg1, dbt1, dg2, dbt2,
                                      dwqkv[C:2 * C], dbqkv[C:2 * C], dwqkv[:C], dbqkv[:C], dwqkv[2 * C:], dbqkv[2 * C:],
                                      dwp, dbp, dw1, db1, dw2, db2]
            saved.layers[i] = None
            if side is None and self.grad_hook is not None:
                self.grad_hook.block_ready(i, bucket(i))
        join_pending()
        dfeats = [torch.empty_like(d) for d in douts]
        dgps = torch.empty(self.B, 2, C, device=dev, dtype=f32)
        dpos = gbuf[L * per_block + 2 * C:].view(1, self.T, C)
        if self._drop("embd") is not None:
            K.dropout_inplace(dx, self._drop("embd"))
        K.tokens_bwd(self.geom, dx, douts if residual else None, dfeats, dgps, dpos)
        grads[0] = dpos
        if self.grad_hook is not None:
            self.grad_hook.finish([gbuf[L * per_block + 2 * C:]])
        return dfeats, dgps, grads

    def _backward_bf16_chain(self, saved, params, douts, dgps_out, residual):
        dev = douts[0].device
        M, C, L, T = self.M, self.C, self.L, self.T
        f32, bf = torch.float32, torch.bfloat16
        F = 4 * C
        grads = [None] * len(params)
        dyf = torch.empty(M, C, device=dev, dtype=f32)
        K.upsample_add_bwd(self.geom, douts, dgps_out, dyf)
        sizes = [3 * C * C, C * C, F * C, C * F, 3 * C, C, F, C, C, C, C, C]
        per_block = sum(sizes)
        gbuf = torch.zeros(L * per_block + 2 * C + self.T * C, device=dev, dtype=f32)

        def block_views(i):
            out, off = [], i * per_block
            for n in sizes:
                out.append(gbuf[off:off + n])
                off += n
            return out

        def bucket(i):
            return gbuf[i * per_block:(i + 1) * per_block + (2 * C if i == L - 1 else 0)]

        env = os.environ.get("DSF_WGRAD_STREAM")
        use_side = (env == "1") if env in ("0", "1") else torch.cuda.is_current_stream_capturing()
        main = torch.cuda.current_stream()
        side = _side_stream(dev) if use_side else None
        side_q = _side_stream(dev, 1) if use_side else None

        def fork(fn, stream=None):
            stream = stream or side
            if stream is None:
                fn()
                return
            ev = torch.cuda.Event()
            ev.record(main)
            stream.wait_event(ev)
            with torch.cuda.stream(stream):
                fn()

        def join(stream):
            if stream is not None:
                ev = torch.cuda.Event()
                ev.record(stream)
                main.wait_event(ev)

        pending = None

        def join_pending():
            nonlocal pending
            if pending is not None:
                ev, blk, _keep = pending
                main.wait_event(ev)
                pending = None
                if self.grad_hook is not None:
                    self.grad_hook.block_ready(blk, bucket(blk))

        def half_b(i, dxa):
            st = saved.layers[i]
            v = block_views(i)
            o = _Ctx()
            o.da = torch.empty(M, F, device=dev, dtype=bf)
            o.dxm = torch.empty(M, C, device=dev, dtype=bf)
            o.dy = torch.empty(M, C, device=dev, dtype=bf)
            o.dx_mid = torch.empty(M, C, device=dev, dtype=f32)
            o.delta = torch.empty(self.B, self.nh, T, device=dev, dtype=f32)
            d = dict(a=st.a, y=st.y, x_mid=st.x_mid, mean2=st.mean2, rstd2=st.rstd2, g2=params[3 + 16 * i], w2_t=st.w2_t, w1_t=st.w1_t,
                     wp_t=st.wp_t, dxa=dxa, da=o.da, dxm=o.dxm, dy=o.dy, dx_mid_out=o.dx_mid, delta=o.delta, db1=v[6], dg2=v[10], dbe2=v[11], dbp=v[5])
            return o, d

        dgf, dbf = gbuf[L * per_block:L * per_block + C], gbuf[L * per_block + C:L * per_block + 2 * C]
        dx = torch.empty(M, C, device=dev, dtype=f32)
        dxa_bufs = [torch.empty(M, C, device=dev, dtype=bf), torch.empty(M, C, device=dev, dtype=bf)]
        K.layernorm_bwd(dyf, saved.x_last, params[-2], saved.mean_f, saved.rstd_f, None, dx, dgf, dbf, dx_bf16=dxa_bufs[(L - 1) & 1],
                        dx_colsum=block_views(L - 1)[7])
        grads[-2], grads[-1] = dgf, dbf
        cur, d = half_b(L - 1, dxa_bufs[(L - 1) & 1])
        K.chain_bwd(M, C, T, self.nh, half_b=d, dx_in=dx)
        dx0 = None
        for i in reversed(range(L)):
            base = 1 + 16 * i
            st = saved.layers[i]
            dxa = dxa_bufs[i & 1]
            dwqkv, dwp, dw1, dw2, dbqkv, dbp, db1, db2, dg1, dbt1, dg2, dbt2 = block_views(i)
            dwqkv, dwp, dw1, dw2 = dwqkv.view(3 * C, C), dwp.view(C, C), dw1.view(F, C), dw2.view(C, F)

            def mlp_proj_wgrads(cur=cur, st=st, dxa=dxa, dw2=dw2, dw1=dw1, dwp=dwp):
                K.gemm_bf16_tn(dxa, st.a, dw2)
                K.gemm_bf16_tn(cur.da, st.h2, dw1)
                K.gemm_bf16_tn(cur.dxm, st.y, dwp)
            fork(mlp_proj_wgrads)
            dqkv = torch.empty(M, 3 * C, device=dev, dtype=bf)
            if side is None:
                K.attn_bwd(st.qkv, st.y, cur.dy, st.lse, cur.delta, dqkv, self.B, T, C, self.nh, None, None, parts=6)
            else:
                fork(lambda: K.attn_bwd(st.qkv, st.y, cur.dy, st.lse, cur.delta, dqkv, self.B, T, C, self.nh, None, None, parts=4), side_q)
                K.attn_bwd(st.qkv, st.y, cur.dy, st.lse, cur.delta, dqkv, self.B, T, C, self.nh, None, None, parts=2)
                join(side_q)
            fork(lambda: K.gemm_bf16_tn(dqkv, st.h1, dwqkv))
            join_pending()
            if side is not None:
                ev_blk = torch.cuda.Event()
                ev_blk.record(side)
                pending = (ev_blk, i, (st, cur, dqkv))
            ha = dict(dqkv=dqkv, dx_mid_in=cur.dx_mid, x_in=st.x_in, mean1=st.mean1, rstd1=st.rstd1, g1=params[base], wqkv_t=st.wqkv_t,
                      dg1=dg1, dbe1=dbt1, dbqkv=dbqkv, db2_prev=block_views(i - 1)[7] if i > 0 else None)
            if i > 0:
                nxt, d = half_b(i - 1, dxa_bufs[(i - 1) & 1])
                K.chain_bwd(M, C, T, self.nh, half_a=ha, half_b=d)
            else:
                nxt = None
                dx0 = torch.empty(M, C, device=dev, dtype=f32)
                K.chain_bwd(M, C, T, self.nh, half_a=ha, dx_f32=dx0)
            grads[base: base + 16] = [dg1, dbt1, dg2, dbt2,
                                      dwqkv[C:2 * C], dbqkv[C:2 * C], dwqkv[:C], dbqkv[:C], dwqkv[2 * C:], dbqkv[2 * C:],
                                      dwp, dbp, dw1, db1, dw2, db2]
            saved.layers[i] = None
            if side is None and self.grad_hook is not None:
                self.grad_hook.block_ready(i, bucket(i))
            cur = nxt
        join_pending()
        dfeats = [torch.empty_like(d_) for d_ in douts]
        dgps = torch.empty(self.B, 2, C, device=dev, dtype=f32)
        dpos = gbuf[L * per_block + 2 * C:].view(1, self.T, C)
        K.tokens_bwd(self.geom, dx0, douts if residual else None, dfeats, dgps, dpos)
        grads[0] = dpos
        if self.grad_hook is not None:
            self.grad_hook.finish([gbuf[L * per_block + 2 * C:]])
        return dfeats, dgps, grads

    def backward(self, saved, params, douts, dgps_out, residual=True):
        if self.bf16:
            if (_chain_mode(self.C, "DSF_CHAIN_BWD", 0) and self.nh == 4 and self.L > 0 and self.dropout is None
                    and params[13].shape[0] == 4 * self.C):
                return self._backward_bf16_chain(saved, params, douts, dgps_out, residual)
            return self._backward_bf16(saved, params, douts, dgps_out, residual)
        dev = douts[0].device
        M, C, L = self.M, self.C, self.L
        f32 = torch.float32
        grads = [None] * len(params)
        dyf = torch.empty(M, C, device=dev, dtype=f32)
        K.upsample_add_bwd(self.geom, douts, dgps_out, dyf)
        dg = torch.zeros(C, device=dev, dtype=f32)
        db = torch.zeros(C, device=dev, dtype=f32)
        dx = torch.empty(M, C, device=dev, dtype=f32)
        K.layernorm_bwd(dyf, saved.x_last, params[-2], saved.mean_f, saved.rstd_f, None, dx, dg, db)
        grads[-2], grads[-1] = dg, db
        for i in reversed(range(L)):
            base = 1 + 16 * i
            (ln1w, ln1b, ln2w, ln2b, kw, kb, qw, qb, vw, vb, pw, pb, w1, b1, w2, b2) = params[base: base + 16]
            st = saved.layers[i]
            da, dw2, db2 = self._linear_bwd(dx, st.a, w2)
            K.relu_bwd(da, st.a)
            dh2, dw1, db1 = self._linear_bwd(da, st.h2, w1)
            dg2 = torch.zeros(C, device=dev, dtype=f32)
            dbt2 = torch.zeros(C, device=dev, dtype=f32)
            dx_mid = torch.empty(M, C, device=dev, dtype=f32)
            K.layernorm_bwd(dh2, st.x_mid, ln2w, st.mean2, st.rstd2, dx, dx_mid, dg2, dbt2)
            dy, dwp, dbp = self._linear_bwd(dx_mid, st.y, pw)
            dqkv = self._attn_bwd(dy, st.qkv, st.y, st)
            dh1, dwqkv, dbqkv = self._linear_bwd(dqkv, st.h1, st.wqkv)
            dg1 = torch.zeros(C, device=dev, dtype=f32)
            dbt1 = torch.zeros(C, device=dev, dtype=f32)
            dx = torch.empty(M, C, device=dev, dtype=f32)
            K.layernorm_bwd(dh1, st.x_in, ln1w, st.mean1, st.rstd1, dx_mid, dx, dg1, dbt1)
            grads[base: base + 16] = [dg1, dbt1, dg2, dbt2,
                                      dwqkv[C:2 * C], dbqkv[C:2 * C], dwqkv[:C], dbqkv[:C], dwqkv[2 * C:], dbqkv[2 * C:],
                                      dwp, dbp, dw1, db1, dw2, db2]
            saved.layers[i] = None
        dfeats = [torch.empty_like(d) for d in douts]
        dgps = torch.empty(self.B, 2, C, device=dev, dtype=f32)
        dpos = torch.empty(1, self.T, C, device=dev, dtype=f32)
        K.tokens_bwd(self.geom, dx, douts if residual else None, dfeats, dgps, dpos)
        grads[0] = dpos
        return dfeats, dgps, grads


def attn_drop_scale(p):
    k = max(1, min(255, int(round(float(p) * 256.0))))
    return 256.0 / (256.0 - k)


def materialise_dropout_masks(dropout, B, T, C, n_head, n_layer, device):
    out = {}

    def elem(kind, blk=0):
        p = float(dropout.get("resid" if kind in ("proj", "mlp") else kind, 0.0))
        if p <= 0.0:
            return None
        m = torch.ones(B, T, C, device=device, dtype=torch.float32)
        sd = dropout.get("seed_dev")
        K.dropout_inplace(m, K.Dropout(p, int(dropout["seed"]), drop_site(kind, blk), int(dropout.get("step", 0)),
                                       None if sd is None else sd.data_ptr()))
        return m

    m = elem("embd")
    if m is not None:
        out["embd"] = m
    for i in range(n_layer):
        for kind in ("proj", "mlp"):
            m = elem(kind, i)
            if m is not None:
                out["%s.%d" % (kind, i)] = m
        if float(dropout.get("attn", 0.0)) > 0.0:
            bits = dropout["capture"]["attn_bits.%d" % i].view(B, n_head, T, -1, 1)
            sh = torch.arange(32, device=device, dtype=torch.int32)
            keep = ((bits >> sh) & 1).reshape(B, n_head, T, -1)[..., :T]
            out["attn.%d" % i] = keep.to(torch.float32) * attn_drop_scale(dropout["attn"])
    return out


def _layout_of(t):
    if t.is_contiguous():
        return K.DSF_NCHW
    if t.dim() == 4 and t.is_contiguous(memory_format=torch.channels_last):
        return K.DSF_NHWC
    raise RuntimeError("feature maps must be contiguous or channels_last")


class FusionStageFn(torch.autograd.Function):

    @staticmethod
    def forward(ctx, cfg, img, lidar, radar, gps_emb, *params):
        for t, n in ((img, "image features"), (lidar, "lidar features"), (radar, "radar features")):
            if not t.is_cuda:
                raise RuntimeError("%s must be CUDA tensors (the fusion stage has no CPU path)" % n)
        for t in (lidar, radar, gps_emb) + tuple(params):
            if t.device != img.device:
                raise RuntimeError("fusion stage: all inputs and parameters must be on %s, found a tensor on %s" % (img.device, t.device))
        with torch.cuda.device(img.device):
            return FusionStageFn._forward(ctx, cfg, img, lidar, radar, gps_emb, *params)

    @staticmethod
    def _forward(ctx, cfg, img, lidar, radar, gps_emb, *params):
        K.check_device()
        layout = _layout_of(img)
        if _layout_of(lidar) != layout or _layout_of(radar) != layout:
            lidar = lidar.contiguous(memory_format=torch.channels_last if layout == K.DSF_NHWC else torch.contiguous_format)
            radar = radar.contiguous(memory_format=torch.channels_last if layout == K.DSF_NHWC else torch.contiguous_format)
        if img.dtype not in (torch.float32, torch.bfloat16) or lidar.dtype != img.dtype or radar.dtype != img.dtype:
            raise RuntimeError("feature maps must share one dtype (float32 or bfloat16)")
        S, V = cfg["seq_len"], cfg["n_views"]
        N, C, H, W = lidar.shape
        B = N // S
        if img.shape[0] != B * V * S or radar.shape[0] != B * S:
            raise RuntimeError("inconsistent frame counts: image %d lidar %d radar %d (seq_len %d, n_views %d)"
                               % (img.shape[0], N, radar.shape[0], S, V))
        r = _Runner(B, S, V, cfg["vert_anchors"], cfg["horz_anchors"], C, H, W, cfg["n_head"], cfg["n_layer"],
                    img.dtype, cfg["compute_dtype"], layout)
        if params[0].shape[1] != r.T:
            raise RuntimeError("pos_emb has %d tokens, inputs imply %d" % (params[0].shape[1], r.T))
        gps_emb = gps_emb.contiguous().float()
        plist = [p.detach().contiguous().float() for p in params]
        residual = bool(cfg.get("residual", True))
        r.grad_hook = cfg.get("grad_hook")
        r.dropout = cfg.get("dropout")
        r.capture = cfg.get("capture")
        r.shadows = cfg.get("shadows")
        if r.dropout is not None and any(float(r.dropout.get(k, 0.0)) > 0.0 for k in ("embd", "attn", "resid")):
            if not r.bf16:
                raise NotImplementedError("dropout is implemented in the bf16 tensor-core mode only (the fp32 mode is the "
                                          "p = 0 parity path)")
        else:
            r.dropout = None
        outs, gps_out, saved = r.forward([img.detach(), lidar.detach(), radar.detach()], gps_emb.detach(), plist, residual)
        ctx.runner, ctx.saved_state, ctx.plist, ctx.residual = r, saved, plist, residual
        ctx.device = img.device
        ctx.param_versions = [p._version for p in params]
        ctx.params_ref = params
        ctx.feat_mf = torch.channels_last if layout == K.DSF_NHWC else torch.contiguous_format
        ctx.gps_dtype = gps_emb.dtype
        return outs[0], outs[1], outs[2], gps_out

    @staticmethod
    @once_differentiable
    def backward(ctx, d_img, d_lidar, d_radar, d_gps):
        if ctx.saved_state is None:
            raise RuntimeError("fusion stage: backward called a second time — the saved activations are released block by block "
                               "during the first backward (retain_graph is not supported; call forward again)")
        if any(p._version != v for p, v in zip(ctx.params_ref, ctx.param_versions)):
            raise RuntimeError("fusion stage: a GPT parameter was modified in place between forward and backward (the bf16 weight "
                               "shadows saved by the forward would no longer match the parameters)")
        with torch.cuda.device(ctx.device):
            return FusionStageFn._backward(ctx, d_img, d_lidar, d_radar, d_gps)

    @staticmethod
    def _backward(ctx, d_img, d_lidar, d_radar, d_gps):
        r = ctx.runner
        mf = ctx.feat_mf

        def prep(d, like_dtype):
            return d.contiguous(memory_format=mf).to(like_dtype)

        fdt = torch.bfloat16 if r.geom.feat_dtype == K.DSF_BF16 else torch.float32
        douts = [prep(d_img, fdt), prep(d_lidar, fdt), prep(d_radar, fdt)]
        dgps_out = None if d_gps is None else d_gps.contiguous().float()
        dfeats, dgps, grads = r.backward(ctx.saved_state, ctx.plist, douts, dgps_out, ctx.residual)
        ctx.saved_state = None
        return (None, dfeats[0], dfeats[1], dfeats[2], dgps) + tuple(grads)


def fusion_stage(cfg, img, lidar, radar, gps_emb, params):
    return FusionStageFn.apply(cfg, img, lidar, radar, gps_emb, *params)


_IMAGENET_MEAN, _IMAGENET_STD = (0.485, 0.456, 0.406), (0.229, 0.224, 0.225)


def stem_pack_supported(frames):
    f0 = frames[0]
    return (0 < len(frames) <= 16 and f0.is_cuda and f0.dim() == 4 and f0.shape[1] <= 3 and (f0.shape[2] * f0.shape[3]) % 4 == 0
            and all(f.is_cuda and f.dtype == torch.float32 and f.shape == f0.shape and f.is_contiguous() and not f.requires_grad
                    and f.device == f0.device for f in frames))


def stem_pack(frames, normalize, dtype, channels_last):
    f0 = frames[0]
    B, Cin, H, W = f0.shape
    with torch.cuda.device(f0.device):
        out = torch.empty((B * len(frames), Cin, H, W), device=f0.device, dtype=dtype,
                          memory_format=torch.channels_last if (channels_last and Cin > 1) else torch.contiguous_format)
        if normalize:
            if Cin != 3:
                raise RuntimeError("normalize_imagenet expects 3-channel frames, got %d channels" % Cin)
            scale = [1.0 / (255.0 * s) for s in _IMAGENET_STD]
            shift = [-m / s for m, s in zip(_IMAGENET_MEAN, _IMAGENET_STD)]
            K.stem_pack(frames, out, scale, shift)
        else:
            K.stem_pack(frames, out)
    return out


class PooledTailFn(torch.autograd.Function):

    @staticmethod
    def forward(ctx, f_img, f_lid, f_rad, gps, B):
        maps = (f_img, f_lid, f_rad)
        ctx.B = B
        ctx.like = maps
        with torch.cuda.device(f_img.device):
            fused = torch.empty((B, f_img.shape[1]), device=f_img.device, dtype=torch.float32)
            K.tail_fwd(maps, gps, fused, B)
        return fused

    @staticmethod
    @once_differentiable
    def backward(ctx, dfused):
        maps = ctx.like
        dfused = dfused.contiguous().float()
        with torch.cuda.device(dfused.device):
            dmaps = [torch.empty_like(m) for m in maps]
            dgps = torch.empty((ctx.B, 2, maps[0].shape[1]), device=dfused.device, dtype=torch.float32)
            K.tail_bwd(dfused, dmaps, dgps, ctx.B)
        return dmaps[0], dmaps[1], dmaps[2], dgps, None


def pooled_tail_supported(f_img, f_lid, f_rad, gps):
    maps = (f_img, f_lid, f_rad)
    lay = K._tail_layout(f_img)
    return (all(m.is_cuda and m.dim() == 4 and m.dtype == f_img.dtype and m.dtype in (torch.float32, torch.bfloat16) and m.shape[1:] == f_img.shape[1:]
                and K._tail_layout(m) == lay and (m.is_contiguous() or m.is_contiguous(memory_format=torch.channels_last)) for m in maps)
            and f_img.shape[1] % 4 == 0 and (f_img.shape[2] * f_img.shape[3]) % 4 == 0
            and gps.is_cuda and gps.dtype == torch.float32 and gps.is_contiguous() and gps.dim() == 3 and gps.shape[1] == 2)


def pooled_tail(f_img, f_lid, f_rad, gps, B):
    return PooledTailFn.apply(f_img, f_lid, f_rad, gps, B)
```

Baseline: 1320.

## Fuse attention backward dK/dV and dQ into one persistent work-item kernel

Replaces the separate dK/dV and dQ backward kernels with a single persistent kernel whose CTAs loop over a flat list of 128-row work items for either role. Barriers and TMEM are set up once per CTA and reused across items through phase-tracked barriers. The Python side drops the second side stream and issues one parts=6 call instead of overlapping two launches. This removes launch and setup overhead and tail imbalance, but adds more complex barrier phase bookkeeping and loses the previous stream-level overlap.

```diff
diff --git a/deepsense6g_tii_b200/csrc/attn_api.cu b/deepsense6g_tii_b200/csrc/attn_api.cu
--- a/deepsense6g_tii_b200/csrc/attn_api.cu
+++ b/deepsense6g_tii_b200/csrc/attn_api.cu
@@ -85,7 +85,7 @@
   if (int e = check_attn_drop("attn_fwd", drop, drop_bits, drop_on)) return e;
   DSF_REQUIRE(B > 0 && T > 0 && C > 0 && nh > 0 && C % nh == 0, "attn_fwd: bad shape B=%d T=%d C=%d nh=%d", B, T, C, nh);
   DSF_REQUIRE(aligned16(qkv) && aligned16(y), "attn_fwd: 16-byte alignment required");
-  DSF_REQUIRE(B <= 65535 && nh <= 65535, "attn_fwd: grid too large");
+  DSF_REQUIRE((int64_t)B * nh * cdiv(T, 128) <= (1 << 30), "attn_fwd: too many 128-row tiles (B=%d nh=%d T=%d)", B, nh, T);
   if (int e = check_head_size("attn_fwd", C / nh)) return e;
   return attn_fwd_run(qkv, y, lse, B, T, C, nh, drop_on ? drop : nullptr, drop_bits, g_attn_impl.load(std::memory_order_relaxed), (cudaStream_t)stream);
 }
@@ -97,7 +97,7 @@
   if (int e = check_attn_drop("attn_bwd", drop, drop_bits, drop_on)) return e;
   DSF_REQUIRE(B > 0 && T > 0 && C > 0 && nh > 0 && C % nh == 0, "attn_bwd: bad shape B=%d T=%d C=%d nh=%d", B, T, C, nh);
   DSF_REQUIRE(aligned16(qkv) && aligned16(y) && aligned16(dy) && aligned16(dqkv), "attn_bwd: 16-byte alignment required");
-  DSF_REQUIRE(B <= 65535 && nh <= 65535, "attn_bwd: grid too large");
+  DSF_REQUIRE((int64_t)B * nh * cdiv(T, 128) <= (1 << 30), "attn_bwd: too many 128-row tiles (B=%d nh=%d T=%d)", B, nh, T);
   if (int e = check_head_size("attn_bwd", C / nh)) return e;
   return attn_bwd_run(qkv, y, dy, lse, delta, dqkv, B, T, C, nh, drop_on ? drop : nullptr, const_cast<uint32_t*>(drop_bits), parts, (cudaStream_t)stream);
 }
diff --git a/deepsense6g_tii_b200/csrc/attn_tc2.cu b/deepsense6g_tii_b200/csrc/attn_tc2.cu
--- a/deepsense6g_tii_b200/csrc/attn_tc2.cu
+++ b/deepsense6g_tii_b200/csrc/attn_tc2.cu
@@ -212,114 +212,133 @@
                    pack_bf16x2(__uint_as_float(a[e + 6]) * scale, __uint_as_float(a[e + 7]) * scale));
 }
 
+struct AttnItem {
+  int b, h, r0;
+};
+__device__ __forceinline__ AttnItem attn_item(int it, int B, int T, int nh, int R) {
+  const int nfull = T / R, n_full_items = B * nh * nfull;
+  int bh, t;
+  if (it < n_full_items) { bh = it / nfull; t = it % nfull; }
+  else { bh = it - n_full_items; t = nfull; }
+  return AttnItem{bh / nh, bh % nh, t * R};
+}
+
 template <int HS, int BQ, int ST, int NP>
 struct BwdKV2 {
   static constexpr int KV_BYTES = 128 * HS * 2, Q_BYTES = BQ * HS * 2;
   static constexpr int K_OFF = 0, V_OFF = KV_BYTES, Q_OFF = 2 * KV_BYTES, DO_OFF = Q_OFF + ST * Q_BYTES;
-  static constexpr int BAR_OFF = DO_OFF + ST * Q_BYTES;
-  static constexpr int NBAR = 2 + 2 * ST + 4;
-  static constexpr int STAT_OFF = BAR_OFF + NBAR * 8 + 16;
+  static constexpr int DATA = DO_OFF + ST * Q_BYTES;
+  static constexpr int NBAR = 3 + 2 * ST + 4;
+  static_assert(4 * BQ + 2 * HS <= 512, "TMEM budget");
+};
+
+template <int HS, int ST>
+struct BwdQ2 {
+  static constexpr int BKV = 64;
+  static constexpr int Q_BYTES = 128 * HS * 2, KV_BYTES = BKV * HS * 2;
+  static constexpr int Q_OFF = 0, DO_OFF = Q_BYTES, K_OFF = 2 * Q_BYTES, V_OFF = K_OFF + ST * KV_BYTES;
+  static constexpr int DATA = V_OFF + ST * KV_BYTES;
+  static constexpr int NBAR = 3 + 2 * ST + 4;
+  static_assert(4 * BKV + 2 * HS <= 512, "TMEM budget (S/dP double-buffered, dQ, Q and dO rows)");
+};
+
+template <int HS, int BQ, int STA, int STB, int NP>
+struct Bwd2 {
+  using KV = BwdKV2<HS, BQ, STA, NP>;
+  using Q = BwdQ2<HS, STB>;
+  static constexpr int KV_BAR = KV::DATA > Q::DATA ? KV::DATA : Q::DATA;
+  static constexpr int Q_BAR = KV_BAR + KV::NBAR * 8;
+  static constexpr int TMEM_SLOT = Q_BAR + Q::NBAR * 8;
+  static constexpr int STAT_OFF = (TMEM_SLOT + 16 + 15) & ~15;
   static constexpr int THREADS = 256 * NP + 64;
-  static_assert(4 * BQ + 2 * HS <= 512, "TMEM budget");
   static_assert(STAT_OFF % 16 == 0, "float4 reads of the statistics");
-  static int dyn_bytes(int T) { return STAT_OFF + 2 * cdiv(T, BQ) * BQ * 4 + 1024; }
+  static int dyn_bytes(int T, bool kv_role) { return STAT_OFF + (kv_role ? 2 * cdiv(T, BQ) * BQ * 4 : 0) + 1024; }
 };
 
+struct BwdArgs {
+  const float* lse;
+  const float* delta;
+  __nv_bfloat16* dqkv;
+  const __nv_bfloat16* qkv;
+  const __nv_bfloat16* dy;
+  int B, T, C, nh;
+  float scale;
+};
+
 template <int HS, int BQ, int ST, int NP, bool DROP, int POLY>
-__global__ void __launch_bounds__(256 * NP + 64, 1)
-attn_bwd_kv2_kernel(const __grid_constant__ CUtensorMap tmKV, const __grid_constant__ CUtensorMap tmQ, const __grid_constant__ CUtensorMap tmDO,
-                    const float* __restrict__ lse, const float* __restrict__ delta, __nv_bfloat16* __restrict__ dqkv, int T, int C, int nh,
-                    float scale, AttnDrop ad) {
+__device__ __noinline__ void bwd_kv_item(const CUtensorMap* tmKV, const CUtensorMap* tmQ, const CUtensorMap* tmDO, const BwdArgs& a,
+                                         const AttnDrop& ad, uint32_t sbase, float* s_lse, uint32_t bar0, uint32_t tmem_base, AttnItem wi,
+                                         int g0, int n) {
   using L = BwdKV2<HS, BQ, ST, NP>;
   constexpr int MMAW = 8 * NP, TMAW = 8 * NP + 1;
-  extern __shared__ uint8_t smem_raw[];
-  const uint32_t sbase = (smem_u32(smem_raw) + 1023u) & ~1023u;
-  uint8_t* smem = smem_raw + (sbase - smem_u32(smem_raw));
-  const uint32_t bar0 = sbase + L::BAR_OFF;
-  const uint32_t kv_full = bar0, acc_done = bar0 + 8, q_full = bar0 + 16, q_empty = q_full + 8 * ST, s_full = q_empty + 8 * ST,
-                 ds_full = s_full + 16, tmem_slot = ds_full + 16;
+  const uint32_t kv_full = bar0, kv_empty = bar0 + 8, acc_done = bar0 + 16, q_full = bar0 + 24, q_empty = q_full + 8 * ST,
+                 s_full = q_empty + 8 * ST, ds_full = s_full + 16;
   const int warp = __shfl_sync(0xffffffffu, (int)(threadIdx.x >> 5), 0), lane = threadIdx.x & 31;
-  const int kv0 = blockIdx.x * 128, h = blockIdx.y, b = blockIdx.z;
+  const int T = a.T, C = a.C, nh = a.nh, kv0 = wi.r0, h = wi.h, b = wi.b;
   const int n_q = (T + BQ - 1) / BQ;
-
-  pdl_trigger();
-  if (threadIdx.x == 0) {
-    mbar_init(kv_full, 1);
-    mbar_init(acc_done, 1);
-    for (int s = 0; s < ST; ++s) { mbar_init(q_full + 8 * s, 1); mbar_init(q_empty + 8 * s, 1); }
-    for (int w = 0; w < 2; ++w) { mbar_init(s_full + 8 * w, 1); mbar_init(ds_full + 8 * w, 256 * NP); }
-    fence_barrier_init();
-  }
-  if (warp == MMAW) { tmem_alloc(tmem_slot, 512); tmem_relinquish(); }
-  if (warp == TMAW && lane == 0) { tma_prefetch_desc(&tmKV); tma_prefetch_desc(&tmQ); tma_prefetch_desc(&tmDO); }
-  tc_fence_before();
-  __syncthreads();
-  tc_fence_after();
-  uint32_t tmem_base;
-  asm volatile("ld.shared.b32 %0, [%1];" : "=r"(tmem_base) : "r"(tmem_slot));
-  pdl_wait();
   const uint32_t tm_dv = tmem_base + 4 * BQ, tm_dk = tm_dv + HS;
 
   if (warp == TMAW) {
     if (lane == 0) {
+      if (n > 0) mbar_wait(kv_empty, (n - 1) & 1);
       mbar_expect_tx(kv_full, 2 * L::KV_BYTES);
-      tma_tile<HS>(sbase + L::K_OFF, &tmKV, kv_full, C + h * HS, kv0, b, 128);
-      tma_tile<HS>(sbase + L::V_OFF, &tmKV, kv_full, 2 * C + h * HS, kv0, b, 128);
+      tma_tile<HS>(sbase + L::K_OFF, tmKV, kv_full, C + h * HS, kv0, b, 128);
+      tma_tile<HS>(sbase + L::V_OFF, tmKV, kv_full, 2 * C + h * HS, kv0, b, 128);
       for (int i = 0; i < n_q; ++i) {
-        const int st = i % ST;
-        if (i >= ST) mbar_wait(q_empty + 8 * st, ((i / ST) - 1) & 1);
+        const int g = g0 + i, st = g % ST;
+        if (g >= ST) mbar_wait(q_empty + 8 * st, ((g / ST) - 1) & 1);
         mbar_expect_tx(q_full + 8 * st, 2 * L::Q_BYTES);
-        tma_tile<HS>(sbase + L::Q_OFF + st * L::Q_BYTES, &tmQ, q_full + 8 * st, h * HS, i * BQ, b, BQ);
-        tma_tile<HS>(sbase + L::DO_OFF + st * L::Q_BYTES, &tmDO, q_full + 8 * st, h * HS, i * BQ, b, BQ);
+        tma_tile<HS>(sbase + L::Q_OFF + st * L::Q_BYTES, tmQ, q_full + 8 * st, h * HS, i * BQ, b, BQ);
+        tma_tile<HS>(sbase + L::DO_OFF + st * L::Q_BYTES, tmDO, q_full + 8 * st, h * HS, i * BQ, b, BQ);
       }
     }
   } else if (warp == MMAW) {
-    {
-      constexpr uint32_t idesc_s = make_idesc_bf16(128, BQ, 0, 0);
-      constexpr uint32_t idesc_g = make_idesc_bf16(128, HS, 0, 1);
-      mbar_wait(kv_full, 0);
-      mbar_wait(q_full, 0);
+    constexpr uint32_t idesc_s = make_idesc_bf16(128, BQ, 0, 0);
+    constexpr uint32_t idesc_g = make_idesc_bf16(128, HS, 0, 1);
+    mbar_wait(kv_full, n & 1);
+    mbar_wait(q_full + 8 * (g0 % ST), (g0 / ST) & 1);
+    tc_fence_after();
+    mma_over_head<HS>(tmem_base + (g0 & 1) * 2 * BQ, sbase + L::K_OFF, 128, sbase + L::Q_OFF + (g0 % ST) * L::Q_BYTES, BQ, idesc_s);
+    mma_over_head<HS>(tmem_base + (g0 & 1) * 2 * BQ + BQ, sbase + L::V_OFF, 128, sbase + L::DO_OFF + (g0 % ST) * L::Q_BYTES, BQ, idesc_s);
+    tc_commit_elect(s_full + 8 * (g0 & 1));
+    if (n_q == 1) tc_commit_elect(kv_empty);
+    for (int i = 0; i < n_q; ++i) {
+      const int g = g0 + i, bf = g & 1, st = g % ST;
+      TRACE(2, i, 0);
+      if (i + 1 < n_q) {
+        const int sn = (g + 1) % ST, bn = (g + 1) & 1;
+        mbar_wait(q_full + 8 * sn, ((g + 1) / ST) & 1);
+        TRACE(2, i, 1);
+        tc_fence_after();
+        mma_over_head<HS>(tmem_base + bn * 2 * BQ, sbase + L::K_OFF, 128, sbase + L::Q_OFF + sn * L::Q_BYTES, BQ, idesc_s);
+        mma_over_head<HS>(tmem_base + bn * 2 * BQ + BQ, sbase + L::V_OFF, 128, sbase + L::DO_OFF + sn * L::Q_BYTES, BQ, idesc_s);
+        tc_commit_elect(s_full + 8 * bn);
+        if (i + 1 == n_q - 1) tc_commit_elect(kv_empty);
+      }
+      TRACE(2, i, 2);
+      mbar_wait(ds_full + 8 * bf, (g >> 1) & 1);
+      TRACE(2, i, 3);
       tc_fence_after();
-      mma_over_head<HS>(tmem_base, sbase + L::K_OFF, 128, sbase + L::Q_OFF, BQ, idesc_s);
-      mma_over_head<HS>(tmem_base + BQ, sbase + L::V_OFF, 128, sbase + L::DO_OFF, BQ, idesc_s);
-      tc_commit_elect(s_full);
-      for (int i = 0; i < n_q; ++i) {
-        const int bf = i & 1, st = i % ST;
-        TRACE(2, i, 0);
-        if (i + 1 < n_q) {
-          const int sn = (i + 1) % ST, bn = (i + 1) & 1;
-          mbar_wait(q_full + 8 * sn, ((i + 1) / ST) & 1);
-          TRACE(2, i, 1);
-          tc_fence_after();
-          mma_over_head<HS>(tmem_base + bn * 2 * BQ, sbase + L::K_OFF, 128, sbase + L::Q_OFF + sn * L::Q_BYTES, BQ, idesc_s);
-          mma_over_head<HS>(tmem_base + bn * 2 * BQ + BQ, sbase + L::V_OFF, 128, sbase + L::DO_OFF + sn * L::Q_BYTES, BQ, idesc_s);
-          tc_commit_elect(s_full + 8 * bn);
-        }
-        TRACE(2, i, 2);
-        mbar_wait(ds_full + 8 * bf, (i >> 1) & 1);
-        TRACE(2, i, 3);
-        tc_fence_after();
-        mma_over_rows_ts<HS, BQ, 32 / NP>(tm_dv, tmem_base + bf * 2 * BQ, sbase + L::DO_OFF + st * L::Q_BYTES, idesc_g, i > 0);
-        mma_over_rows_ts<HS, BQ, 32 / NP>(tm_dk, tmem_base + bf * 2 * BQ + BQ, sbase + L::Q_OFF + st * L::Q_BYTES, idesc_g, i > 0);
-        tc_commit_elect(q_empty + 8 * st);
-        TRACE(2, i, 4);
-      }
-      tc_commit_elect(acc_done);
-    }
+      mma_over_rows_ts<HS, BQ, 32 / NP>(tm_dv, tmem_base + bf * 2 * BQ, sbase + L::DO_OFF + st * L::Q_BYTES, idesc_g, i > 0);
+      mma_over_rows_ts<HS, BQ, 32 / NP>(tm_dk, tmem_base + bf * 2 * BQ + BQ, sbase + L::Q_OFF + st * L::Q_BYTES, idesc_g, i > 0);
+      tc_commit_elect(q_empty + 8 * st);
+      TRACE(2, i, 4);
+    }
+    tc_commit_elect(acc_done);
   } else {
     constexpr int CW = BQ / (2 * NP);
     const int wgi = warp >> 2;
     const int row = (warp & 3) * 32 + lane;
     const uint32_t lane_off = (uint32_t)((warp & 3) * 32) << 16;
     const bool key_ok = (kv0 + row) < T;
-    const float scale_log2 = scale * 1.4426950408889634f;
-    const float* lse_g = lse + ((size_t)b * nh + h) * T;
-    const float* delta_g = delta + ((size_t)b * nh + h) * T;
+    const float scale_log2 = a.scale * 1.4426950408889634f;
+    const float* lse_g = a.lse + ((size_t)b * nh + h) * T;
+    const float* delta_g = a.delta + ((size_t)b * nh + h) * T;
     static_assert(BQ == 64 && (CW == 32 || CW == 16), "a 64-query tile in 32- or 16-column shares");
     const size_t bh = (size_t)b * nh + h;
     const int kw = kv0 / 32 + (warp & 3);
-    float* s_lse = reinterpret_cast<float*>(smem + L::STAT_OFF);
     float* s_delta = s_lse + n_q * BQ;
+    if (n > 0) named_bar_sync(1, 256 * NP);
     for (int idx = threadIdx.x; idx < n_q * BQ; idx += 256 * NP) {
       s_lse[idx] = idx < T ? __ldg(lse_g + idx) * -1.4426950408889634f : -INFINITY;
       s_delta[idx] = idx < T ? -__ldg(delta_g + idx) : 0.f;
@@ -332,14 +351,14 @@
     if (DROP) fetch_w(0);
     named_bar_sync(1, 256 * NP);
     for (int i = 0; i < n_q; ++i) {
-      const int bf = i & 1;
+      const int g = g0 + i, bf = g & 1;
       const float* wst = s_lse + i * BQ + wgi * CW;
       const float* wsd = s_delta + i * BQ + wgi * CW;
       const uint32_t myw = wv;
       if ((warp & 3) == 0 && wgi < 2) TRACE(wgi, i, 0);
       if (DROP && i + 1 < n_q) fetch_w(i + 1);
       if ((warp & 3) == 0 && wgi < 2) TRACE(wgi, i, 1);
-      mbar_wait(s_full + 8 * bf, (i >> 1) & 1);
+      mbar_wait(s_full + 8 * bf, (g >> 1) & 1);
       if ((warp & 3) == 0 && wgi < 2) TRACE(wgi, i, 2);
       tc_fence_after();
       const uint32_t tm_s = tmem_base + bf * 2 * BQ + lane_off + wgi * CW, tm_dp = tm_s + BQ;
@@ -394,10 +413,10 @@
       mbar_arrive(ds_full + 8 * bf);
       if ((warp & 3) == 0 && wgi < 2) TRACE(wgi, i, 5);
     }
-    mbar_wait(acc_done, 0);
+    mbar_wait(acc_done, n & 1);
     tc_fence_after();
     const int ld = 3 * C;
-    __nv_bfloat16* dk_row = dqkv + ((size_t)b * T + kv0 + row) * ld + C + h * HS;
+    __nv_bfloat16* dk_row = a.dqkv + ((size_t)b * T + kv0 + row) * ld + C + h * HS;
     __nv_bfloat16* dv_row = dk_row + C;
     constexpr int NSPLIT = (NP == 2 && HS >= 32) ? 2 : 1;
     constexpr int CH = HS / NSPLIT;
@@ -405,119 +424,80 @@
     if (part < NSPLIT) {
 #pragma unroll 1
       for (int c = part * CH; c < (part + 1) * CH; c += 16) {
-        uint32_t a[16];
-        tmem_ld16((which == 0 ? tm_dk : tm_dv) + lane_off + c, a);
+        uint32_t v[16];
+        tmem_ld16((which == 0 ? tm_dk : tm_dv) + lane_off + c, v);
         tmem_wait_ld();
-        if (key_ok) store_row16_bf16((which == 0 ? dk_row : dv_row) + c, a, which == 0 ? scale : 1.0f);
-      }
-    }
-  }
-  tc_fence_before();
-  __syncthreads();
-  if (warp == MMAW) tmem_dealloc(tmem_base, 512);
-}
-
-template <int HS, int ST>
-struct BwdQ2 {
-  static constexpr int BKV = 64;
-  static constexpr int Q_BYTES = 128 * HS * 2, KV_BYTES = BKV * HS * 2;
-  static constexpr int Q_OFF = 0, DO_OFF = Q_BYTES, K_OFF = 2 * Q_BYTES, V_OFF = K_OFF + ST * KV_BYTES;
-  static constexpr int BAR_OFF = V_OFF + ST * KV_BYTES;
-  static constexpr int NBAR = 2 + 2 * ST + 4;
-  static constexpr int DYN = BAR_OFF + NBAR * 8 + 16 + 1024;
-  static_assert(4 * BKV + HS <= 512, "TMEM budget");
-};
+        if (key_ok) store_row16_bf16((which == 0 ? dk_row : dv_row) + c, v, which == 0 ? a.scale : 1.0f);
+      }
+    }
+    tc_fence_before();
+  }
+}
 
 template <int HS, int ST, bool AT, int NP, bool DROP, int POLY>
-__global__ void __launch_bounds__(256 * NP + 64, 1)
-attn_bwd_q2_kernel(const __grid_constant__ CUtensorMap tmQ, const __grid_constant__ CUtensorMap tmDO, const __grid_constant__ CUtensorMap tmKV,
-                   const float* __restrict__ lse, const float* __restrict__ delta, __nv_bfloat16* __restrict__ dqkv, int T, int C, int nh,
-                   float scale, AttnDrop ad, const __nv_bfloat16* __restrict__ qkv, const __nv_bfloat16* __restrict__ dy) {
+__device__ __noinline__ void bwd_q_item(const CUtensorMap* tmQ, const CUtensorMap* tmDO, const CUtensorMap* tmKV, const BwdArgs& a,
+                                        const AttnDrop& ad, uint32_t sbase, uint32_t bar0, uint32_t kv_acc_done, uint32_t tmem_base, AttnItem wi,
+                                        int g0, int n, int kv_items) {
   using L = BwdQ2<HS, ST>;
   constexpr int BKV = L::BKV;
   constexpr int MMAW = 8 * NP, TMAW = 8 * NP + 1;
-  extern __shared__ uint8_t smem_raw[];
-  const uint32_t sbase = (smem_u32(smem_raw) + 1023u) & ~1023u;
-  const uint32_t bar0 = sbase + L::BAR_OFF;
-  const uint32_t q_full = bar0, acc_done = bar0 + 8, kv_full = bar0 + 16, kv_empty = kv_full + 8 * ST, s_full = kv_empty + 8 * ST,
-                 ds_full = s_full + 16, tmem_slot = ds_full + 16;
+  const uint32_t q_full = bar0, q_empty = bar0 + 8, acc_done = bar0 + 16, kv_full = bar0 + 24, kv_empty = kv_full + 8 * ST,
+                 s_full = kv_empty + 8 * ST, ds_full = s_full + 16;
   const int warp = __shfl_sync(0xffffffffu, (int)(threadIdx.x >> 5), 0), lane = threadIdx.x & 31;
-  const int q0 = blockIdx.x * 128, h = blockIdx.y, b = blockIdx.z;
+  const int T = a.T, C = a.C, nh = a.nh, q0 = wi.r0, h = wi.h, b = wi.b;
   const int n_kv = (T + BKV - 1) / BKV;
-  constexpr uint32_t TMEM_COLS = (4 * BKV + HS + (AT ? (HS >= 32 ? HS : 32) : 0)) <= 256 ? 256 : 512;
-  static_assert(4 * BKV + 2 * HS <= 512, "TMEM budget (S/dP double-buffered, dQ, Q and dO rows)");
-
-  pdl_trigger();
-  if (threadIdx.x == 0) {
-    mbar_init(q_full, AT ? 256 : 1);
-    mbar_init(acc_done, 1);
-    for (int s = 0; s < ST; ++s) { mbar_init(kv_full + 8 * s, 1); mbar_init(kv_empty + 8 * s, 1); }
-    for (int w = 0; w < 2; ++w) { mbar_init(s_full + 8 * w, 1); mbar_init(ds_full + 8 * w, 256 * NP); }
-    fence_barrier_init();
-  }
-  if (warp == MMAW) { tmem_alloc(tmem_slot, TMEM_COLS); tmem_relinquish(); }
-  if (warp == TMAW && lane == 0) { tma_prefetch_desc(&tmKV); tma_prefetch_desc(&tmQ); tma_prefetch_desc(&tmDO); }
-  tc_fence_before();
-  __syncthreads();
-  tc_fence_after();
-  uint32_t tmem_base;
-  asm volatile("ld.shared.b32 %0, [%1];" : "=r"(tmem_base) : "r"(tmem_slot));
-  pdl_wait();
   const uint32_t tm_dq = tmem_base + 4 * BKV;
   const uint32_t tm_q = tm_dq + HS, tm_do = tm_q + (HS >= 32 ? HS / 2 : 16);
 
   if (warp == TMAW) {
     if (lane == 0) {
+      if (n == 0 && kv_items > 0) mbar_wait(kv_acc_done, (kv_items - 1) & 1);
       if (!AT) {
+        if (n > 0) mbar_wait(q_empty, (n - 1) & 1);
         mbar_expect_tx(q_full, 2 * L::Q_BYTES);
-        tma_tile<HS>(sbase + L::Q_OFF, &tmQ, q_full, h * HS, q0, b, 128);
-        tma_tile<HS>(sbase + L::DO_OFF, &tmDO, q_full, h * HS, q0, b, 128);
+        tma_tile<HS>(sbase + L::Q_OFF, tmQ, q_full, h * HS, q0, b, 128);
+        tma_tile<HS>(sbase + L::DO_OFF, tmDO, q_full, h * HS, q0, b, 128);
       }
       for (int j = 0; j < n_kv; ++j) {
-        const int st = j % ST;
-        if (j >= ST) mbar_wait(kv_empty + 8 * st, ((j / ST) - 1) & 1);
+        const int g = g0 + j, st = g % ST;
+        if (g >= ST) mbar_wait(kv_empty + 8 * st, ((g / ST) - 1) & 1);
         mbar_expect_tx(kv_full + 8 * st, 2 * L::KV_BYTES);
-        tma_tile<HS>(sbase + L::K_OFF + st * L::KV_BYTES, &tmKV, kv_full + 8 * st, C + h * HS, j * BKV, b, BKV);
-        tma_tile<HS>(sbase + L::V_OFF + st * L::KV_BYTES, &tmKV, kv_full + 8 * st, 2 * C + h * HS, j * BKV, b, BKV);
+        tma_tile<HS>(sbase + L::K_OFF + st * L::KV_BYTES, tmKV, kv_full + 8 * st, C + h * HS, j * BKV, b, BKV);
+        tma_tile<HS>(sbase + L::V_OFF + st * L::KV_BYTES, tmKV, kv_full + 8 * st, 2 * C + h * HS, j * BKV, b, BKV);
       }
     }
   } else if (warp == MMAW) {
-    {
-      constexpr uint32_t idesc_s = make_idesc_bf16(128, BKV, 0, 0);
-      constexpr uint32_t idesc_q = make_idesc_bf16(128, HS, 0, 1);
-      mbar_wait(q_full, 0);
-      mbar_wait(kv_full, 0);
+    constexpr uint32_t idesc_s = make_idesc_bf16(128, BKV, 0, 0);
+    constexpr uint32_t idesc_q = make_idesc_bf16(128, HS, 0, 1);
+    auto issue_s = [&](int g) {
+      const int s = g % ST, bb = g & 1;
+      if (AT) {
+        mma_over_head_ts<HS>(tmem_base + bb * 2 * BKV, tm_q, sbase + L::K_OFF + s * L::KV_BYTES, BKV, idesc_s);
+        mma_over_head_ts<HS>(tmem_base + bb * 2 * BKV + BKV, tm_do, sbase + L::V_OFF + s * L::KV_BYTES, BKV, idesc_s);
+      } else {
+        mma_over_head<HS>(tmem_base + bb * 2 * BKV, sbase + L::Q_OFF, 128, sbase + L::K_OFF + s * L::KV_BYTES, BKV, idesc_s);
+        mma_over_head<HS>(tmem_base + bb * 2 * BKV + BKV, sbase + L::DO_OFF, 128, sbase + L::V_OFF + s * L::KV_BYTES, BKV, idesc_s);
+      }
+      tc_commit_elect(s_full + 8 * bb);
+      if (!AT && g == g0 + n_kv - 1) tc_commit_elect(q_empty);
+    };
+    mbar_wait(q_full, n & 1);
+    mbar_wait(kv_full + 8 * (g0 % ST), (g0 / ST) & 1);
+    tc_fence_after();
+    issue_s(g0);
+    for (int j = 0; j < n_kv; ++j) {
+      const int g = g0 + j, bf = g & 1, st = g % ST;
+      if (j + 1 < n_kv) {
+        mbar_wait(kv_full + 8 * ((g + 1) % ST), ((g + 1) / ST) & 1);
+        tc_fence_after();
+        issue_s(g + 1);
+      }
+      mbar_wait(ds_full + 8 * bf, (g >> 1) & 1);
       tc_fence_after();
-      if (AT) {
-        mma_over_head_ts<HS>(tmem_base, tm_q, sbase + L::K_OFF, BKV, idesc_s);
-        mma_over_head_ts<HS>(tmem_base + BKV, tm_do, sbase + L::V_OFF, BKV, idesc_s);
-      } else {
-        mma_over_head<HS>(tmem_base, sbase + L::Q_OFF, 128, sbase + L::K_OFF, BKV, idesc_s);
-        mma_over_head<HS>(tmem_base + BKV, sbase + L::DO_OFF, 128, sbase + L::V_OFF, BKV, idesc_s);
-      }
-      tc_commit_elect(s_full);
-      for (int j = 0; j < n_kv; ++j) {
-        const int bf = j & 1, st = j % ST;
-        if (j + 1 < n_kv) {
-          const int sn = (j + 1) % ST, bn = (j + 1) & 1;
-          mbar_wait(kv_full + 8 * sn, ((j + 1) / ST) & 1);
-          tc_fence_after();
-          if (AT) {
-            mma_over_head_ts<HS>(tmem_base + bn * 2 * BKV, tm_q, sbase + L::K_OFF + sn * L::KV_BYTES, BKV, idesc_s);
-            mma_over_head_ts<HS>(tmem_base + bn * 2 * BKV + BKV, tm_do, sbase + L::V_OFF + sn * L::KV_BYTES, BKV, idesc_s);
-          } else {
-            mma_over_head<HS>(tmem_base + bn * 2 * BKV, sbase + L::Q_OFF, 128, sbase + L::K_OFF + sn * L::KV_BYTES, BKV, idesc_s);
-            mma_over_head<HS>(tmem_base + bn * 2 * BKV + BKV, sbase + L::DO_OFF, 128, sbase + L::V_OFF + sn * L::KV_BYTES, BKV, idesc_s);
-          }
-          tc_commit_elect(s_full + 8 * bn);
-        }
-        mbar_wait(ds_full + 8 * bf, (j >> 1) & 1);
-        tc_fence_after();
-        mma_over_rows_ts<HS, BKV, 32 / NP>(tm_dq, tmem_base + bf * 2 * BKV + BKV, sbase + L::K_OFF + st * L::KV_BYTES, idesc_q, j > 0);
-        tc_commit_elect(kv_empty + 8 * st);
-      }
-      tc_commit_elect(acc_done);
-    }
+      mma_over_rows_ts<HS, BKV, 32 / NP>(tm_dq, tmem_base + bf * 2 * BKV + BKV, sbase + L::K_OFF + st * L::KV_BYTES, idesc_q, j > 0);
+      tc_commit_elect(kv_empty + 8 * st);
+    }
+    tc_commit_elect(acc_done);
   } else {
     constexpr int CW = BKV / (2 * NP);
     static_assert(BKV == 64 && (CW == 32 || CW == 16), "a 64-key tile in 32- or 16-column shares");
@@ -526,34 +506,37 @@
     const uint32_t lane_off = (uint32_t)((warp & 3) * 32) << 16;
     const int q = q0 + row;
     const bool q_ok = q < T;
-    const float scale_log2 = scale * 1.4426950408889634f;
-    const float my_lse = q_ok ? lse[((size_t)b * nh + h) * T + q] * 1.4426950408889634f : INFINITY;
-    const float my_delta = q_ok ? delta[((size_t)b * nh + h) * T + q] : 0.f;
-    if (AT && wgi < 2) {
-      const __nv_bfloat16* src = wgi == 0 ? qkv + ((size_t)b * T + q) * (3 * C) + h * HS : dy + ((size_t)b * T + q) * C + h * HS;
-      const uint32_t dst = (wgi == 0 ? tm_q : tm_do) + lane_off;
+    const float scale_log2 = a.scale * 1.4426950408889634f;
+    const float my_lse = q_ok ? a.lse[((size_t)b * nh + h) * T + q] * 1.4426950408889634f : INFINITY;
+    const float my_delta = q_ok ? a.delta[((size_t)b * nh + h) * T + q] : 0.f;
+    if (AT) {
+      if (n == 0 && kv_items > 0) named_bar_sync(2, 256 * NP);
+      if (wgi < 2) {
+        const __nv_bfloat16* src = wgi == 0 ? a.qkv + ((size_t)b * T + q) * (3 * C) + h * HS : a.dy + ((size_t)b * T + q) * C + h * HS;
+        const uint32_t dst = (wgi == 0 ? tm_q : tm_do) + lane_off;
 #pragma unroll 1
-      for (int c = 0; c < HS; c += 32) {
-        uint32_t wds[16];
-#pragma unroll
-        for (int k = 0; k < 4; ++k) {
-          const bool real = q_ok && (HS >= 32 || k < 2);
-          const uint4 v = real ? __ldg(reinterpret_cast<const uint4*>(src + c) + k) : make_uint4(0u, 0u, 0u, 0u);
-          wds[4 * k] = v.x; wds[4 * k + 1] = v.y; wds[4 * k + 2] = v.z; wds[4 * k + 3] = v.w;
+        for (int c = 0; c < HS; c += 32) {
+          uint32_t wds[16];
+#pragma unroll
+          for (int k = 0; k < 4; ++k) {
+            const bool real = q_ok && (HS >= 32 || k < 2);
+            const uint4 v = real ? __ldg(reinterpret_cast<const uint4*>(src + c) + k) : make_uint4(0u, 0u, 0u, 0u);
+            wds[4 * k] = v.x; wds[4 * k + 1] = v.y; wds[4 * k + 2] = v.z; wds[4 * k + 3] = v.w;
+          }
+          tmem_st16(dst + c / 2, wds);
         }
-        tmem_st16(dst + c / 2, wds);
-      }
-      tmem_wait_st();
-      tc_fence_before();
-      mbar_arrive(q_full);
+        tmem_wait_st();
+        tc_fence_before();
+        mbar_arrive(q_full);
+      }
     }
     const uint32_t* my_bits = (DROP && q_ok) ? ad.bits + (((size_t)b * nh + h) * T + q) * ad.Tw + (wgi * CW) / 32 : nullptr;
     uint32_t wnext = my_bits ? my_bits[0] : 0xFFFFFFFFu;
     for (int j = 0; j < n_kv; ++j) {
-      const int bf = j & 1, kv0 = j * BKV;
+      const int g = g0 + j, bf = g & 1, kv0 = j * BKV;
       const uint32_t keepw = wnext >> ((wgi * CW) % 32);
       if (my_bits && j + 1 < n_kv) wnext = my_bits[2 * (j + 1)];
-      mbar_wait(s_full + 8 * bf, (j >> 1) & 1);
+      mbar_wait(s_full + 8 * bf, (g >> 1) & 1);
       tc_fence_after();
       const uint32_t tm_s = tmem_base + bf * 2 * BKV + lane_off + wgi * CW, tm_dp = tm_s + BKV;
       const bool full = kv0 + BKV <= T;
@@ -593,25 +576,83 @@
       tc_fence_before();
       mbar_arrive(ds_full + 8 * bf);
     }
-    mbar_wait(acc_done, 0);
+    mbar_wait(acc_done, n & 1);
     tc_fence_after();
-    __nv_bfloat16* dq_row = dqkv + ((size_t)b * T + q) * (3 * C) + h * HS;
+    __nv_bfloat16* dq_row = a.dqkv + ((size_t)b * T + q) * (3 * C) + h * HS;
     constexpr int NG = (HS / 16) < 2 * NP ? (HS / 16) : 2 * NP;
     constexpr int CH = HS / NG;
-    const int g = wgi;
-    if (g < NG) {
+    const int gi = wgi;
+    if (gi < NG) {
 #pragma unroll 1
-      for (int c = g * CH; c < (g + 1) * CH; c += 16) {
-        uint32_t a[16];
-        tmem_ld16(tm_dq + lane_off + c, a);
+      for (int c = gi * CH; c < (gi + 1) * CH; c += 16) {
+        uint32_t v[16];
+        tmem_ld16(tm_dq + lane_off + c, v);
         tmem_wait_ld();
-        if (q_ok) store_row16_bf16(dq_row + c, a, scale);
-      }
-    }
+        if (q_ok) store_row16_bf16(dq_row + c, v, a.scale);
+      }
+    }
+    tc_fence_before();
+  }
+}
+
+template <int HS, int BQ, int STA, int STB, bool AT, int NP, bool DROP, int POLY>
+__global__ void __launch_bounds__(256 * NP + 64, 1)
+attn_bwd2_kernel(const __grid_constant__ CUtensorMap tmKV128, const __grid_constant__ CUtensorMap tmQs, const __grid_constant__ CUtensorMap tmDOs,
+                 const __grid_constant__ CUtensorMap tmQ128, const __grid_constant__ CUtensorMap tmDO128, const __grid_constant__ CUtensorMap tmKV64,
+                 const BwdArgs a, AttnDrop ad, int roles) {
+  using L = Bwd2<HS, BQ, STA, STB, NP>;
+  constexpr int MMAW = 8 * NP, TMAW = 8 * NP + 1;
+  extern __shared__ uint8_t smem_raw[];
+  const uint32_t sbase = (smem_u32(smem_raw) + 1023u) & ~1023u;
+  float* s_stat = reinterpret_cast<float*>(smem_raw + (sbase - smem_u32(smem_raw)) + L::STAT_OFF);
+  const uint32_t kv_bar = sbase + L::KV_BAR, q_bar = sbase + L::Q_BAR, tmem_slot = sbase + L::TMEM_SLOT;
+  const int warp = __shfl_sync(0xffffffffu, (int)(threadIdx.x >> 5), 0), lane = threadIdx.x & 31;
+  const int tiles = a.B * a.nh * ((a.T + 127) / 128);
+  const int n_kv_items = (roles & 2) ? tiles : 0;
+  const int n_items = n_kv_items + ((roles & 4) ? tiles : 0);
+
+  pdl_trigger();
+  if (threadIdx.x == 0) {
+    mbar_init(kv_bar, 1);
+    mbar_init(kv_bar + 8, 1);
+    mbar_init(kv_bar + 16, 1);
+    for (int s = 0; s < STA; ++s) { mbar_init(kv_bar + 24 + 8 * s, 1); mbar_init(kv_bar + 24 + 8 * STA + 8 * s, 1); }
+    for (int w = 0; w < 2; ++w) { mbar_init(kv_bar + 24 + 16 * STA + 8 * w, 1); mbar_init(kv_bar + 40 + 16 * STA + 8 * w, 256 * NP); }
+    mbar_init(q_bar, AT ? 256 : 1);
+    mbar_init(q_bar + 8, 1);
+    mbar_init(q_bar + 16, 1);
+    for (int s = 0; s < STB; ++s) { mbar_init(q_bar + 24 + 8 * s, 1); mbar_init(q_bar + 24 + 8 * STB + 8 * s, 1); }
+    for (int w = 0; w < 2; ++w) { mbar_init(q_bar + 24 + 16 * STB + 8 * w, 1); mbar_init(q_bar + 40 + 16 * STB + 8 * w, 256 * NP); }
+    fence_barrier_init();
+  }
+  if (warp == MMAW) { tmem_alloc(tmem_slot, 512); tmem_relinquish(); }
+  if (warp == TMAW && lane == 0) {
+    tma_prefetch_desc(&tmKV128); tma_prefetch_desc(&tmQs); tma_prefetch_desc(&tmDOs);
+    tma_prefetch_desc(&tmQ128); tma_prefetch_desc(&tmDO128); tma_prefetch_desc(&tmKV64);
   }
   tc_fence_before();
   __syncthreads();
-  if (warp == MMAW) tmem_dealloc(tmem_base, TMEM_COLS);
+  tc_fence_after();
+  uint32_t tmem_base;
+  asm volatile("ld.shared.b32 %0, [%1];" : "=r"(tmem_base) : "r"(tmem_slot));
+  pdl_wait();
+
+  const int n_q = (a.T + BQ - 1) / BQ, n_kv = (a.T + BwdQ2<HS, STB>::BKV - 1) / BwdQ2<HS, STB>::BKV;
+  int kv_g = 0, kv_n = 0, q_g = 0, q_n = 0;
+  for (int it = blockIdx.x; it < n_items; it += gridDim.x) {
+    if (it < n_kv_items) {
+      bwd_kv_item<HS, BQ, STA, NP, DROP, POLY>(&tmKV128, &tmQs, &tmDOs, a, ad, sbase, s_stat, kv_bar, tmem_base, attn_item(it, a.B, a.T, a.nh, 128), kv_g, kv_n);
+      kv_g += n_q;
+      ++kv_n;
+    } else {
+      bwd_q_item<HS, STB, AT, NP, DROP, POLY>(&tmQ128, &tmDO128, &tmKV64, a, ad, sbase, q_bar, kv_bar + 16, tmem_base, attn_item(it - n_kv_items, a.B, a.T, a.nh, 128), q_g, q_n, kv_n);
+      q_g += n_kv;
+      ++q_n;
+    }
+  }
+  tc_fence_before();
+  __syncthreads();
+  if (warp == MMAW) tmem_dealloc(tmem_base, 512);
 }
 
 template <int HS, int KST, int VST, int NWG = 2, bool PT = false>
@@ -620,7 +661,7 @@
   static constexpr int Q_BYTES = 128 * HS * 2, KV_BYTES = BKV * HS * 2, P_BYTES = 128 * BKV * 2;
   static constexpr int Q_OFF = 0, K_OFF = NWG * Q_BYTES, V_OFF = K_OFF + KST * KV_BYTES, P_OFF = V_OFF + VST * KV_BYTES;
   static constexpr int BAR_OFF = P_OFF + (PT ? 0 : 2 * NWG * P_BYTES);
-  static constexpr int NBAR = 1 + 2 * KST + 2 * VST + 12;
+  static constexpr int NBAR = 2 + 2 * KST + 2 * VST + 12;
   static constexpr int DYN = BAR_OFF + NBAR * 8 + 16 + 1024;
   static constexpr int THREADS = 128 * NWG + 64;
   static constexpr int MIN_CTAS = NWG == 1 ? 2 : 1;
@@ -632,7 +673,7 @@
 template <int HS, int KST, int VST, bool PT, bool PP, int NWG = 2, int POLY = 0>
 __global__ void __launch_bounds__(128 * NWG + 64, NWG == 1 ? 2 : 1)
 attn_fwd3_kernel(const __grid_constant__ CUtensorMap tmQ, const __grid_constant__ CUtensorMap tmKV, __nv_bfloat16* __restrict__ y,
-                 float* __restrict__ lse, int T, int C, int nh, float scale_log2, AttnDrop ad) {
+                 float* __restrict__ lse, int B, int T, int C, int nh, float scale_log2, AttnDrop ad) {
   using L = Fwd3<HS, KST, VST, NWG, PT>;
   constexpr int BKV = L::BKV;
   constexpr int MMAW = 4 * NWG, TMAW = 4 * NWG + 1;
@@ -641,15 +682,16 @@
   const uint32_t sbase = (smem_u32(smem_raw) + 1023u) & ~1023u;
   uint8_t* smem = smem_raw + (sbase - smem_u32(smem_raw));
   const uint32_t bar0 = sbase + L::BAR_OFF;
-  const uint32_t q_full = bar0, k_full = bar0 + 8, k_empty = k_full + 8 * KST, v_full = k_empty + 8 * KST, v_empty = v_full + 8 * VST,
-                 s_full = v_empty + 8 * VST, p_full = s_full + 32, p_empty = p_full + 32, tmem_slot = p_empty + 32;
+  const uint32_t q_full = bar0, q_empty = bar0 + 8, k_full = bar0 + 16, k_empty = k_full + 8 * KST, v_full = k_empty + 8 * KST,
+                 v_empty = v_full + 8 * VST, s_full = v_empty + 8 * VST, p_full = s_full + 32, p_empty = p_full + 32, tmem_slot = p_empty + 32;
   const int warp = __shfl_sync(0xffffffffu, (int)(threadIdx.x >> 5), 0), lane = threadIdx.x & 31;
-  const int q0 = blockIdx.x * (128 * NWG), h = blockIdx.y, b = blockIdx.z;
   const int n_kv = (T + BKV - 1) / BKV;
+  const int n_items = B * nh * ((T + 128 * NWG - 1) / (128 * NWG));
 
   pdl_trigger();
   if (threadIdx.x == 0) {
     mbar_init(q_full, 1);
+    mbar_init(q_empty, 1);
     for (int s = 0; s < KST; ++s) { mbar_init(k_full + 8 * s, 1); mbar_init(k_empty + 8 * s, 1); }
     for (int s = 0; s < VST; ++s) { mbar_init(v_full + 8 * s, 1); mbar_init(v_empty + 8 * s, 1); }
     for (int i = 0; i < 2 * NWG; ++i) { mbar_init(s_full + 8 * i, 1); mbar_init(p_full + 8 * i, 128); mbar_init(p_empty + 8 * i, 1); }
@@ -671,41 +713,49 @@
 
   if (warp == TMAW) {
     if (lane == 0) {
-      mbar_expect_tx(q_full, NWG * L::Q_BYTES);
-      for (int w = 0; w < NWG; ++w) tma_tile<HS>(sbase + L::Q_OFF + w * L::Q_BYTES, &tmQ, q_full, h * HS, q0 + 128 * w, b, 128);
-      for (int j = 0; j < n_kv; ++j) {
-        const int ks = j % KST, vs = j % VST;
-        if (j >= KST) mbar_wait(k_empty + 8 * ks, ((j / KST) - 1) & 1);
-        mbar_expect_tx(k_full + 8 * ks, L::KV_BYTES);
-        tma_tile<HS>(sbase + L::K_OFF + ks * L::KV_BYTES, &tmKV, k_full + 8 * ks, C + h * HS, j * BKV, b, BKV);
-        if (j >= VST) mbar_wait(v_empty + 8 * vs, ((j / VST) - 1) & 1);
-        mbar_expect_tx(v_full + 8 * vs, L::KV_BYTES);
-        tma_tile<HS>(sbase + L::V_OFF + vs * L::KV_BYTES, &tmKV, v_full + 8 * vs, 2 * C + h * HS, j * BKV, b, BKV);
+      int g0 = 0, n = 0;
+      for (int it = blockIdx.x; it < n_items; it += gridDim.x, g0 += n_kv, ++n) {
+        const AttnItem wi = attn_item(it, B, T, nh, 128 * NWG);
+        if (n > 0) mbar_wait(q_empty, (n - 1) & 1);
+        mbar_expect_tx(q_full, NWG * L::Q_BYTES);
+        for (int w = 0; w < NWG; ++w) tma_tile<HS>(sbase + L::Q_OFF + w * L::Q_BYTES, &tmQ, q_full, wi.h * HS, wi.r0 + 128 * w, wi.b, 128);
+        for (int j = 0; j < n_kv; ++j) {
+          const int g = g0 + j, ks = g % KST, vs = g % VST;
+          if (g >= KST) mbar_wait(k_empty + 8 * ks, ((g / KST) - 1) & 1);
+          mbar_expect_tx(k_full + 8 * ks, L::KV_BYTES);
+          tma_tile<HS>(sbase + L::K_OFF + ks * L::KV_BYTES, &tmKV, k_full + 8 * ks, C + wi.h * HS, j * BKV, wi.b, BKV);
+          if (g >= VST) mbar_wait(v_empty + 8 * vs, ((g / VST) - 1) & 1);
+          mbar_expect_tx(v_full + 8 * vs, L::KV_BYTES);
+          tma_tile<HS>(sbase + L::V_OFF + vs * L::KV_BYTES, &tmKV, v_full + 8 * vs, 2 * C + wi.h * HS, j * BKV, wi.b, BKV);
+        }
       }
     }
   } else if (warp == MMAW) {
-    {
-      constexpr uint32_t idesc_s = make_idesc_bf16(128, BKV, 0, 0);
-      constexpr uint32_t idesc_o = make_idesc_bf16(128, HS, 0, 1);
-      mbar_wait(q_full, 0);
+    constexpr uint32_t idesc_s = make_idesc_bf16(128, BKV, 0, 0);
+    constexpr uint32_t idesc_o = make_idesc_bf16(128, HS, 0, 1);
+    int g0 = 0, n = 0;
+    for (int it = blockIdx.x; it < n_items; it += gridDim.x, g0 += n_kv, ++n) {
+      mbar_wait(q_full, n & 1);
       for (int jj = 0; jj < 2 && jj < n_kv; ++jj) {
-        mbar_wait(k_full + 8 * (jj % KST), (jj / KST) & 1);
+        const int g = g0 + jj;
+        mbar_wait(k_full + 8 * (g % KST), (g / KST) & 1);
         tc_fence_after();
         for (int w = 0; w < NWG; ++w) {
-          mma_over_head<HS>(tmem_base + (w * 2 + jj) * BKV, sbase + L::Q_OFF + w * L::Q_BYTES, 128, sbase + L::K_OFF + (jj % KST) * L::KV_BYTES,
+          mma_over_head<HS>(tmem_base + (w * 2 + (g & 1)) * BKV, sbase + L::Q_OFF + w * L::Q_BYTES, 128, sbase + L::K_OFF + (g % KST) * L::KV_BYTES,
                             BKV, idesc_s);
-          tc_commit_elect(s_full + 8 * (w * 2 + jj));
+          tc_commit_elect(s_full + 8 * (w * 2 + (g & 1)));
         }
-        tc_commit_elect(k_empty + 8 * (jj % KST));
+        tc_commit_elect(k_empty + 8 * (g % KST));
+        if (jj == n_kv - 1) tc_commit_elect(q_empty);
       }
       for (int j = 0; j < n_kv; ++j) {
-        const int buf = j & 1, vs = j % VST;
+        const int g = g0 + j, buf = g & 1, vs = g % VST;
         TRACE(2, j, 0);
-        mbar_wait(v_full + 8 * vs, (j / VST) & 1);
+        mbar_wait(v_full + 8 * vs, (g / VST) & 1);
         for (int w = 0; w < NWG; ++w) {
           const int sb = w * 2 + buf;
           TRACE(2, j, 1 + 2 * w);
-          mbar_wait(p_full + 8 * sb, (j >> 1) & 1);
+          mbar_wait(p_full + 8 * sb, (g >> 1) & 1);
           TRACE(2, j, 2 + 2 * w);
           tc_fence_after();
           if (PT)
@@ -716,11 +766,14 @@
           tc_commit_elect(p_empty + 8 * sb);
           if (w == NWG - 1) tc_commit_elect(v_empty + 8 * vs);
           if (j + 2 < n_kv) {
-            const int ks = (j + 2) % KST;
-            if (w == 0) { mbar_wait(k_full + 8 * ks, ((j + 2) / KST) & 1); tc_fence_after(); }
+            const int ks = (g + 2) % KST;
+            if (w == 0) { mbar_wait(k_full + 8 * ks, ((g + 2) / KST) & 1); tc_fence_after(); }
             mma_over_head<HS>(tmem_base + sb * BKV, sbase + L::Q_OFF + w * L::Q_BYTES, 128, sbase + L::K_OFF + ks * L::KV_BYTES, BKV, idesc_s);
             tc_commit_elect(s_full + 8 * sb);
-            if (w == NWG - 1) tc_commit_elect(k_empty + 8 * ks);
+            if (w == NWG - 1) {
+              tc_commit_elect(k_empty + 8 * ks);
+              if (j + 2 == n_kv - 1) tc_commit_elect(q_empty);
+            }
           }
         }
       }
@@ -730,140 +783,146 @@
     const int row = (warp & 3) * 32 + lane;
     const uint32_t lane_off = (uint32_t)((warp & 3) * 32) << 16;
     const uint32_t tm_o = tmem_base + 2 * NWG * BKV + w * HS + lane_off;
-    float m_run = -INFINITY, l_run = 0.f;
     if (PP && w == 1) named_bar_arrive(3, 256);
-    for (int j = 0; j < n_kv; ++j) {
-      const int kv0 = j * BKV, buf = j & 1, sb = w * 2 + buf;
-      const uint32_t tm_s = tmem_base + sb * BKV + lane_off;
-      uint8_t* p_tile = smem + L::P_OFF + sb * L::P_BYTES;
-      if ((warp & 3) == 0) TRACE(w, j, 0);
-      mbar_wait(s_full + 8 * sb, (j >> 1) & 1);
-      if ((warp & 3) == 0) TRACE(w, j, 1);
-      tc_fence_after();
-      uint32_t r0[32], r1[32];
-      tmem_ld32(tm_s, r0);
-      tmem_ld32(tm_s + 32, r1);
-      tmem_wait_ld();
-      if ((warp & 3) == 0) TRACE(w, j, 2);
-      float p_max = -INFINITY;
-      if (kv0 + BKV <= T) {
-        float m4[4] = {-INFINITY, -INFINITY, -INFINITY, -INFINITY};
-#pragma unroll
-        for (int i = 0; i < 32; ++i) m4[i & 3] = fmaxf(m4[i & 3], fmaxf(__uint_as_float(r0[i]), __uint_as_float(r1[i])));
-        p_max = fmaxf(fmaxf(m4[0], m4[1]), fmaxf(m4[2], m4[3]));
-      } else {
-#pragma unroll
-        for (int i = 0; i < 32; ++i) {
-          if (kv0 + i < T) p_max = fmaxf(p_max, __uint_as_float(r0[i]));
-          if (kv0 + 32 + i < T) p_max = fmaxf(p_max, __uint_as_float(r1[i]));
+    int g0 = 0;
+    for (int it = blockIdx.x; it < n_items; it += gridDim.x, g0 += n_kv) {
+      const AttnItem wi = attn_item(it, B, T, nh, 128 * NWG);
+      const int b = wi.b, h = wi.h, q0 = wi.r0;
+      float m_run = -INFINITY, l_run = 0.f;
+      for (int j = 0; j < n_kv; ++j) {
+        const int g = g0 + j, kv0 = j * BKV, buf = g & 1, sb = w * 2 + buf;
+        const uint32_t tm_s = tmem_base + sb * BKV + lane_off;
+        uint8_t* p_tile = smem + L::P_OFF + sb * L::P_BYTES;
+        if ((warp & 3) == 0) TRACE(w, j, 0);
+        mbar_wait(s_full + 8 * sb, (g >> 1) & 1);
+        if ((warp & 3) == 0) TRACE(w, j, 1);
+        tc_fence_after();
+        uint32_t r0[32], r1[32];
+        tmem_ld32(tm_s, r0);
+        tmem_ld32(tm_s + 32, r1);
+        tmem_wait_ld();
+        if ((warp & 3) == 0) TRACE(w, j, 2);
+        float p_max = -INFINITY;
+        if (kv0 + BKV <= T) {
+          float m4[4] = {-INFINITY, -INFINITY, -INFINITY, -INFINITY};
+#pragma unroll
+          for (int i = 0; i < 32; ++i) m4[i & 3] = fmaxf(m4[i & 3], fmaxf(__uint_as_float(r0[i]), __uint_as_float(r1[i])));
+          p_max = fmaxf(fmaxf(m4[0], m4[1]), fmaxf(m4[2], m4[3]));
+        } else {
+#pragma unroll
+          for (int i = 0; i < 32; ++i) {
+            if (kv0 + i < T) p_max = fmaxf(p_max, __uint_as_float(r0[i]));
+            if (kv0 + 32 + i < T) p_max = fmaxf(p_max, __uint_as_float(r1[i]));
+          }
         }
-      }
-      p_max *= scale_log2;
-      const bool need = p_max > m_run + 8.f;
-      if (__any_sync(0xffffffffu, need)) {
-        const float m_new = need ? p_max : m_run;
-        const float alpha = ex2_approx(m_run - m_new);
-        if (j > 0) {
-          mbar_wait(p_empty + 8 * (w * 2 + ((j - 1) & 1)), ((j - 1) >> 1) & 1);
-          tc_fence_after();
+        p_max *= scale_log2;
+        const bool need = p_max > m_run + 8.f;
+        if (__any_sync(0xffffffffu, need)) {
+          const float m_new = need ? p_max : m_run;
+          const float alpha = ex2_approx(m_run - m_new);
+          if (j > 0) {
+            mbar_wait(p_empty + 8 * (w * 2 + ((g - 1) & 1)), ((g - 1) >> 1) & 1);
+            tc_fence_after();
 #pragma unroll 1
-          for (int c = 0; c < HS; c += 16) {
-            uint32_t o[16];
-            tmem_ld16(tm_o + c, o);
-            tmem_wait_ld();
-#pragma unroll
-            for (int i = 0; i < 16; ++i) o[i] = __float_as_uint(__uint_as_float(o[i]) * alpha);
-            tmem_st16(tm_o + c, o);
+            for (int c = 0; c < HS; c += 16) {
+              uint32_t o[16];
+              tmem_ld16(tm_o + c, o);
+              tmem_wait_ld();
+#pragma unroll
+              for (int i = 0; i < 16; ++i) o[i] = __float_as_uint(__uint_as_float(o[i]) * alpha);
+              tmem_st16(tm_o + c, o);
+            }
+            tmem_wait_st();
           }
-          tmem_wait_st();
+          l_run *= alpha;
+          m_run = m_new;
         }
-        l_run *= alpha;
-        m_run = m_new;
-      }
-      if ((warp & 3) == 0) TRACE(w, j, 3);
-      if (!PT && j >= 2) mbar_wait(p_empty + 8 * sb, ((j >> 1) - 1) & 1);
-      if (PP) named_bar_sync(3 + w, 256);
-      if ((warp & 3) == 0) TRACE(w, j, 4);
-      float l_add = 0.f;
-      const bool full = kv0 + BKV <= T;
-      const int qrow = q0 + 128 * w + row;
-      const uint64_t rowid = ((uint64_t)b * nh + h) * T + qrow;
-      if (POLY > 0 && PT && full && !ad.thresh8) {
-        const uint64_t sc2 = pack2(scale_log2, scale_log2), nm2 = pack2(-m_run, -m_run);
-        uint64_t lsum = pack2(0.f, 0.f);
+        if ((warp & 3) == 0) TRACE(w, j, 3);
+        if (!PT && g >= 2) mbar_wait(p_empty + 8 * sb, ((g >> 1) - 1) & 1);
+        if (PP) named_bar_sync(3 + w, 256);
+        if ((warp & 3) == 0) TRACE(w, j, 4);
+        float l_add = 0.f;
+        const bool full = kv0 + BKV <= T;
+        const int qrow = q0 + 128 * w + row;
+        const uint64_t rowid = ((uint64_t)b * nh + h) * T + qrow;
+        if (POLY > 0 && PT && full && !ad.thresh8) {
+          const uint64_t sc2 = pack2(scale_log2, scale_log2), nm2 = pack2(-m_run, -m_run);
+          uint64_t lsum = pack2(0.f, 0.f);
+#pragma unroll
+          for (int half = 0; half < 2; ++half) {
+            uint32_t pk[16];
+#pragma unroll
+            for (int i = 0; i < 32; i += 2) {
+              const uint32_t a0 = half ? r1[i] : r0[i], a1 = half ? r1[i + 1] : r0[i + 1];
+              const uint64_t x = fma2(pack2(__uint_as_float(a0), __uint_as_float(a1)), sc2, nm2);
+              float p0, p1;
+              if (((i / 2) % (POLY > 0 ? POLY : 1)) == POLY - 1) {
+                ex2_poly2(x, p0, p1);
+              } else {
+                float x0, x1;
+                unpack2(x, x0, x1);
+                p0 = ex2_approx(x0);
+                p1 = ex2_approx(x1);
+              }
+              lsum = add2(lsum, pack2(p0, p1));
+              pk[i / 2] = pack_bf16x2(p0, p1);
+            }
+            tmem_st16(tm_s + half * 16, pk);
+          }
+          float l0, l1;
+          unpack2(lsum, l0, l1);
+          l_add = l0 + l1;
+        } else
 #pragma unroll
         for (int half = 0; half < 2; ++half) {
+          uint32_t keepw = 0xFFFFFFFFu;
+          if (ad.thresh8) {
+            keepw = attn_keep_word(ad, rowid, (uint32_t)(kv0 / 32 + half));
+            if (qrow < T) ad.bits[rowid * ad.Tw + kv0 / 32 + half] = keepw;
+          }
           uint32_t pk[16];
 #pragma unroll
           for (int i = 0; i < 32; i += 2) {
             const uint32_t a0 = half ? r1[i] : r0[i], a1 = half ? r1[i + 1] : r0[i + 1];
-            const uint64_t x = fma2(pack2(__uint_as_float(a0), __uint_as_float(a1)), sc2, nm2);
-            float p0, p1;
-            if (((i / 2) % (POLY > 0 ? POLY : 1)) == POLY - 1) {
-              ex2_poly2(x, p0, p1);
-            } else {
-              float x0, x1;
-              unpack2(x, x0, x1);
-              p0 = ex2_approx(x0);
-              p1 = ex2_approx(x1);
+            float p0 = ex2_approx(fmaf(__uint_as_float(a0), scale_log2, -m_run));
+            float p1 = ex2_approx(fmaf(__uint_as_float(a1), scale_log2, -m_run));
+            if (!full) {
+              if (kv0 + half * 32 + i >= T) p0 = 0.f;
+              if (kv0 + half * 32 + i + 1 >= T) p1 = 0.f;
             }
-            lsum = add2(lsum, pack2(p0, p1));
+            l_add += p0 + p1;
+            if (ad.thresh8) {
+              p0 *= (keepw >> i) & 1u ? ad.scale : 0.f;
+              p1 *= (keepw >> (i + 1)) & 1u ? ad.scale : 0.f;
+            }
             pk[i / 2] = pack_bf16x2(p0, p1);
           }
-          tmem_st16(tm_s + half * 16, pk);
+          if (PT) tmem_st16(tm_s + half * 16, pk);
+          else store_p32<BKV>(p_tile, row, half * 32, pk);
         }
-        float l0, l1;
-        unpack2(lsum, l0, l1);
-        l_add = l0 + l1;
-      } else
-#pragma unroll
-      for (int half = 0; half < 2; ++half) {
-        uint32_t keepw = 0xFFFFFFFFu;
-        if (ad.thresh8) {
-          keepw = attn_keep_word(ad, rowid, (uint32_t)(kv0 / 32 + half));
-          if (qrow < T) ad.bits[rowid * ad.Tw + kv0 / 32 + half] = keepw;
-        }
-        uint32_t pk[16];
-#pragma unroll
-        for (int i = 0; i < 32; i += 2) {
-          const uint32_t a0 = half ? r1[i] : r0[i], a1 = half ? r1[i + 1] : r0[i + 1];
-          float p0 = ex2_approx(fmaf(__uint_as_float(a0), scale_log2, -m_run));
-          float p1 = ex2_approx(fmaf(__uint_as_float(a1), scale_log2, -m_run));
-          if (!full) {
-            if (kv0 + half * 32 + i >= T) p0 = 0.f;
-            if (kv0 + half * 32 + i + 1 >= T) p1 = 0.f;
-          }
-          l_add += p0 + p1;
-          if (ad.thresh8) {
-            p0 *= (keepw >> i) & 1u ? ad.scale : 0.f;
-            p1 *= (keepw >> (i + 1)) & 1u ? ad.scale : 0.f;
-          }
-          pk[i / 2] = pack_bf16x2(p0, p1);
-        }
-        if (PT) tmem_st16(tm_s + half * 16, pk);
-        else store_p32<BKV>(p_tile, row, half * 32, pk);
-      }
-      if (PP) named_bar_arrive(4 - w, 256);
-      l_run += l_add;
-      if (PT) tmem_wait_st();
-      else fence_proxy_async();
-      tc_fence_before();
-      mbar_arrive(p_full + 8 * sb);
-      if ((warp & 3) == 0) TRACE(w, j, 5);
-    }
-    mbar_wait(p_empty + 8 * (w * 2 + ((n_kv - 1) & 1)), ((n_kv - 1) >> 1) & 1);
-    tc_fence_after();
-    const int q = q0 + 128 * w + row;
-    const float inv_l = 1.0f / l_run;
-    __nv_bfloat16* yrow = y + ((size_t)b * T + q) * C + h * HS;
+        if (PP) named_bar_arrive(4 - w, 256);
+        l_run += l_add;
+        if (PT) tmem_wait_st();
+        else fence_proxy_async();
+        tc_fence_before();
+        mbar_arrive(p_full + 8 * sb);
+        if ((warp & 3) == 0) TRACE(w, j, 5);
+      }
+      const int gl = g0 + n_kv - 1;
+      mbar_wait(p_empty + 8 * (w * 2 + (gl & 1)), (gl >> 1) & 1);
+      tc_fence_after();
+      const int q = q0 + 128 * w + row;
+      const float inv_l = 1.0f / l_run;
+      __nv_bfloat16* yrow = y + ((size_t)b * T + q) * C + h * HS;
 #pragma unroll 1
-    for (int c = 0; c < HS; c += 16) {
-      uint32_t o[16];
-      tmem_ld16(tm_o + c, o);
-      tmem_wait_ld();
-      if (q < T) store_row16_bf16(yrow + c, o, inv_l);
-    }
-    if (q < T) lse[((size_t)b * nh + h) * T + q] = (m_run + log2f(l_run)) * 0.6931471805599453f;
+      for (int c = 0; c < HS; c += 16) {
+        uint32_t o[16];
+        tmem_ld16(tm_o + c, o);
+        tmem_wait_ld();
+        if (q < T) store_row16_bf16(yrow + c, o, inv_l);
+      }
+      if (q < T) lse[((size_t)b * nh + h) * T + q] = (m_run + log2f(l_run)) * 0.6931471805599453f;
+    }
   }
   tc_fence_before();
   __syncthreads();
@@ -915,9 +974,10 @@
   if (int e = make_tmap3(&tmQ, qkv, 3 * C, T, B, H::BOXC, 128)) return e;
   if (int e = make_tmap3(&tmKV, qkv, 3 * C, T, B, H::BOXC, L::BKV)) return e;
   const float scale_log2 = (1.0f / sqrtf((float)HS)) * 1.4426950408889634f;
-  dim3 grid(cdiv(T, 128 * NWG), nh, B);
-  launch_pdl(attn_fwd3_kernel<HS, KST, VST, true, false, NWG, POLY>, grid, dim3(L::THREADS), L::DYN, st, tmQ, tmKV, (__nv_bfloat16*)y, lse, T, C, nh,
-             scale_log2, ad);
+  const int items = B * nh * cdiv(T, 128 * NWG);
+  const dim3 grid(std::min(items, L::MIN_CTAS * num_sms()));
+  launch_pdl(attn_fwd3_kernel<HS, KST, VST, true, false, NWG, POLY>, grid, dim3(L::THREADS), L::DYN, st, tmQ, tmKV, (__nv_bfloat16*)y, lse, B, T, C,
+             nh, scale_log2, ad);
   return check_launch("attn_fwd3");
 }
 
@@ -934,72 +994,49 @@
 static const bool g_attn_a_in_tmem = getenv("DSF_ATTN_A_TMEM") ? atoi(getenv("DSF_ATTN_A_TMEM")) != 0 : true;
 constexpr int kBwdPairs = 1;
 
-template <int HS, int BQ, int STA, int NP, bool DROP, int POLY>
-static int launch_bwd_kv(const CUtensorMap& tmKV128, const CUtensorMap& tmQs, const CUtensorMap& tmDOs, const float* lse, const float* delta, void* dqkv,
-                         dim3 grid, int T, int C, int nh, float scale, const AttnDrop& ad, cudaStream_t st) {
-  using LA = BwdKV2<HS, BQ, STA, NP>;
-  const int dyn = LA::dyn_bytes(T);
-  if (dyn > 232448) { set_error("attn_bwd: T = %d needs %d bytes of shared memory for the per-query statistics (limit 232448)", T, dyn); return DSF_EUNSUPPORTED; }
+template <int HS, int BQ, int STA, int STB, bool AT, bool DROP>
+static int launch_bwd2k(const CUtensorMap (&tm)[6], const BwdArgs& args, const AttnDrop& ad, int roles, cudaStream_t st) {
+  using L = Bwd2<HS, BQ, STA, STB, kBwdPairs>;
+  auto kernel = attn_bwd2_kernel<HS, BQ, STA, STB, AT, kBwdPairs, DROP, 0>;
+  const int dyn = L::dyn_bytes(args.T, roles & 2);
+  if (dyn > 232448) {
+    set_error("attn_bwd: T = %d needs %d bytes of shared memory for the per-query statistics (limit 232448)", args.T, dyn);
+    return DSF_EUNSUPPORTED;
+  }
   static bool configured_on[64] = {};
   bool& configured = per_device_flag(configured_on);
   if (!configured) {
-    if (cudaFuncSetAttribute(attn_bwd_kv2_kernel<HS, BQ, STA, NP, DROP, POLY>, cudaFuncAttributeMaxDynamicSharedMemorySize, 232448) != cudaSuccess)
-      return check_launch("attn_bwd2/kv/attr");
+    if (cudaFuncSetAttribute(kernel, cudaFuncAttributeMaxDynamicSharedMemorySize, 232448) != cudaSuccess) return check_launch("attn_bwd2/attr");
     configured = true;
   }
-  launch_pdl(attn_bwd_kv2_kernel<HS, BQ, STA, NP, DROP, POLY>, grid, dim3(LA::THREADS), dyn, st, tmKV128, tmQs, tmDOs, lse, delta, (__nv_bfloat16*)dqkv, T, C,
-             nh, scale, ad);
-  return check_launch("attn_bwd2/kv");
-}
-
-template <int HS, int STB, bool AT, int NP, bool DROP, int POLY>
-static int launch_bwd_q(const CUtensorMap& tmQ128, const CUtensorMap& tmDO128, const CUtensorMap& tmKV64, const float* lse, const float* delta, void* dqkv,
-                        dim3 grid, int T, int C, int nh, float scale, const AttnDrop& ad, const void* qkv, const void* dy, cudaStream_t st) {
-  using LB = BwdQ2<HS, STB>;
-  static bool configured_on[64] = {};
-  bool& configured = per_device_flag(configured_on);
-  if (!configured) {
-    if (cudaFuncSetAttribute(attn_bwd_q2_kernel<HS, STB, AT, NP, DROP, POLY>, cudaFuncAttributeMaxDynamicSharedMemorySize, LB::DYN) != cudaSuccess)
-      return check_launch("attn_bwd2/q/attr");
-    configured = true;
-  }
-  launch_pdl(attn_bwd_q2_kernel<HS, STB, AT, NP, DROP, POLY>, grid, dim3(256 * NP + 64), LB::DYN, st, tmQ128, tmDO128, tmKV64, lse, delta, (__nv_bfloat16*)dqkv, T,
-             C, nh, scale, ad, (const __nv_bfloat16*)qkv, (const __nv_bfloat16*)dy);
-  return check_launch("attn_bwd2/q");
+  const int items = ((roles & 2) ? 1 : 0) + ((roles & 4) ? 1 : 0);
+  const int n_items = items * args.B * args.nh * cdiv(args.T, 128);
+  launch_pdl(kernel, dim3(std::min(n_items, num_sms())), dim3(L::THREADS), dyn, st, tm[0], tm[1], tm[2], tm[3], tm[4], tm[5], args, ad, roles);
+  return check_launch("attn_bwd2");
 }
 
 template <int HS, int BQ, int STA, int STB>
 static int launch_bwd2(const void* qkv, const void* y, const void* dy, const float* lse, float* delta, void* dqkv, int B, int T, int C, int nh,
                        const AttnDrop& ad, int parts, cudaStream_t st) {
   using H = HeadCfg<HS>;
-  const float scale = 1.0f / sqrtf((float)HS);
   if (parts & 1) {
     if (int e = run_attn_delta(y, dy, delta, B, T, C, nh, st)) return e;
   }
-  const dim3 grid(cdiv(T, 128), nh, B);
+  const int roles = parts & 6;
+  if (!roles) return DSF_OK;
+  CUtensorMap tm[6];
+  if (int e = make_tmap3(&tm[0], qkv, 3 * C, T, B, H::BOXC, 128)) return e;
+  if (int e = make_tmap3(&tm[1], qkv, 3 * C, T, B, H::BOXC, BQ)) return e;
+  if (int e = make_tmap3(&tm[2], dy, C, T, B, H::BOXC, BQ)) return e;
+  if (int e = make_tmap3(&tm[3], qkv, 3 * C, T, B, H::BOXC, 128)) return e;
+  if (int e = make_tmap3(&tm[4], dy, C, T, B, H::BOXC, 128)) return e;
+  if (int e = make_tmap3(&tm[5], qkv, 3 * C, T, B, H::BOXC, 64)) return e;
+  const BwdArgs args{lse, delta, (__nv_bfloat16*)dqkv, (const __nv_bfloat16*)qkv, (const __nv_bfloat16*)dy, B, T, C, nh, 1.0f / sqrtf((float)HS)};
   const bool drop = ad.thresh8 != 0;
-  if (parts & 2) {
-    CUtensorMap tmKV128, tmQs, tmDOs;
-    if (int e = make_tmap3(&tmKV128, qkv, 3 * C, T, B, H::BOXC, 128)) return e;
-    if (int e = make_tmap3(&tmQs, qkv, 3 * C, T, B, H::BOXC, BQ)) return e;
-    if (int e = make_tmap3(&tmDOs, dy, C, T, B, H::BOXC, BQ)) return e;
-#define DSF_KV(DROP) launch_bwd_kv<HS, BQ, STA, kBwdPairs, DROP, 0>(tmKV128, tmQs, tmDOs, lse, (const float*)delta, dqkv, grid, T, C, nh, scale, ad, st)
-    if (int e = drop ? DSF_KV(true) : DSF_KV(false)) return e;
-#undef DSF_KV
-  }
-  if (parts & 4) {
-    CUtensorMap tmQ128, tmDO128, tmKV64;
-    if (int e = make_tmap3(&tmQ128, qkv, 3 * C, T, B, H::BOXC, 128)) return e;
-    if (int e = make_tmap3(&tmDO128, dy, C, T, B, H::BOXC, 128)) return e;
-    if (int e = make_tmap3(&tmKV64, qkv, 3 * C, T, B, H::BOXC, 64)) return e;
-#define DSF_Q(AT, DROP) launch_bwd_q<HS, STB, AT, kBwdPairs, DROP, 0>(tmQ128, tmDO128, tmKV64, lse, (const float*)delta, dqkv, grid, T, C, nh, scale, ad, qkv, dy, st)
-    int e;
-    if (g_attn_a_in_tmem) e = drop ? DSF_Q(true, true) : DSF_Q(true, false);
-    else e = drop ? DSF_Q(false, true) : DSF_Q(false, false);
-#undef DSF_Q
-    if (e) return e;
-  }
-  return DSF_OK;
+#define DSF_BWD(AT, DROP) launch_bwd2k<HS, BQ, STA, STB, AT, DROP>(tm, args, ad, roles, st)
+  if (g_attn_a_in_tmem) return drop ? DSF_BWD(true, true) : DSF_BWD(true, false);
+  return drop ? DSF_BWD(false, true) : DSF_BWD(false, false);
+#undef DSF_BWD
 }
 
 #ifdef DSF_ATTN_TRACE
diff --git a/deepsense6g_tii_b200/functional.py b/deepsense6g_tii_b200/functional.py
--- a/deepsense6g_tii_b200/functional.py
+++ b/deepsense6g_tii_b200/functional.py
@@ -31,8 +31,8 @@
 _SIDE_STREAMS = {}
 
 
-def _side_stream(device, which=0):
-    key = (device.type, device.index, which)
+def _side_stream(device):
+    key = (device.type, device.index)
     if key not in _SIDE_STREAMS:
         _SIDE_STREAMS[key] = torch.cuda.Stream(device=device)
     return _SIDE_STREAMS[key]
@@ -336,25 +336,16 @@
         use_side = (env == "1") if env in ("0", "1") else torch.cuda.is_current_stream_capturing()
         main = torch.cuda.current_stream()
         side = _side_stream(dev) if use_side else None
-        side_q = _side_stream(dev, 1) if use_side else None
-
-        def fork(fn, stream=None):
-            stream = stream or side
-            if stream is None:
+
+        def fork(fn):
+            if side is None:
                 fn()
                 return
             ev = torch.cuda.Event()
             ev.record(main)
-            stream.wait_event(ev)
-            with torch.cuda.stream(stream):
+            side.wait_event(ev)
+            with torch.cuda.stream(side):
                 fn()
-
-        def join(stream=None):
-            stream = stream or side
-            if stream is not None:
-                ev = torch.cuda.Event()
-                ev.record(stream)
-                main.wait_event(ev)
 
         pending = None
 
@@ -404,9 +395,7 @@
             else:
                 adrop = self._drop("attn", i)
                 K.attn_bwd(st.qkv, st.y, dy, st.lse, delta, dqkv, self.B, self.T, C, self.nh, adrop, st.drop_bits, parts=1)
-                fork(lambda: K.attn_bwd(st.qkv, st.y, dy, st.lse, delta, dqkv, self.B, self.T, C, self.nh, adrop, st.drop_bits, parts=4), side_q)
-                K.attn_bwd(st.qkv, st.y, dy, st.lse, delta, dqkv, self.B, self.T, C, self.nh, adrop, st.drop_bits, parts=2)
-                join(side_q)
+                K.attn_bwd(st.qkv, st.y, dy, st.lse, delta, dqkv, self.B, self.T, C, self.nh, adrop, st.drop_bits, parts=6)
 
             fork(lambda: K.gemm_bf16_tn(dqkv, st.h1, dwqkv, colsum=dbqkv))
             dh1 = torch.empty(M, C, device=dev, dtype=dh_dt)
@@ -465,24 +454,16 @@
         use_side = (env == "1") if env in ("0", "1") else torch.cuda.is_current_stream_capturing()
         main = torch.cuda.current_stream()
         side = _side_stream(dev) if use_side else None
-        side_q = _side_stream(dev, 1) if use_side else None
-
-        def fork(fn, stream=None):
-            stream = stream or side
-            if stream is None:
+
+        def fork(fn):
+            if side is None:
                 fn()
                 return
             ev = torch.cuda.Event()
             ev.record(main)
-            stream.wait_event(ev)
-            with torch.cuda.stream(stream):
+            side.wait_event(ev)
+            with torch.cuda.stream(side):
                 fn()
-
-        def join(stream):
-            if stream is not None:
-                ev = torch.cuda.Event()
-                ev.record(stream)
-                main.wait_event(ev)
 
         pending = None
 
@@ -530,12 +511,7 @@
                 K.gemm_bf16_tn(cur.dxm, st.y, dwp)
             fork(mlp_proj_wgrads)
             dqkv = torch.empty(M, 3 * C, device=dev, dtype=bf)
-            if side is None:
-                K.attn_bwd(st.qkv, st.y, cur.dy, st.lse, cur.delta, dqkv, self.B, T, C, self.nh, None, None, parts=6)
-            else:
-                fork(lambda: K.attn_bwd(st.qkv, st.y, cur.dy, st.lse, cur.delta, dqkv, self.B, T, C, self.nh, None, None, parts=4), side_q)
-                K.attn_bwd(st.qkv, st.y, cur.dy, st.lse, cur.delta, dqkv, self.B, T, C, self.nh, None, None, parts=2)
-                join(side_q)
+            K.attn_bwd(st.qkv, st.y, cur.dy, st.lse, cur.delta, dqkv, self.B, T, C, self.nh, None, None, parts=6)
             fork(lambda: K.gemm_bf16_tn(dqkv, st.h1, dwqkv))
             join_pending()
             if side is not None:
```

Result: slower. 1261, median of 6 (-4.5%).
